# Sahar-E/NeRF-and-DietNeRF

Hardware: AMD Instinct MI355X
Metric: rays/sec (coarse+fine) at 256x256, 64 coarse + 128 fine samples (higher is better)
Workload: dtype f16 (3-pass hi/lo split operands, f32 accumulate; fp32-class results)

## Files before the change

nerf_and_dietnerf_amd/csrc/mlp_f16_frag.h:

```cpp
#pragma once
#include "mlp_common.h"

namespace nerf {

typedef _Float16 h8 __attribute__((ext_vector_type(8)));
typedef _Float16 h2 __attribute__((ext_vector_type(2)));
typedef uint32_t frag4 __attribute__((ext_vector_type(4)));

template <int OFF>
__device__ __forceinline__ void lds_read_frag_asm(f32x4& dst, uint32_t base) {
    asm volatile("ds_read_b128 %0, %1 offset:%2" : "=a"(dst) : "v"(base), "n"(OFF) : "memory");
}
template <int N>
__device__ __forceinline__ void lds_wait_frag_asm(f32x4& reg) {
#ifdef NERF_DIAG_NO_LDSWAIT
    asm volatile("" : "+a"(reg) : : "memory");
#else
    asm volatile("s_waitcnt lgkmcnt(%1)" : "+a"(reg) : "n"(N) : "memory");
#endif
}

__device__ __forceinline__ uint32_t pack_h2(float a, float b) {
    const h2 t = {(_Float16)a, (_Float16)b};
    return __builtin_bit_cast(uint32_t, t);
}

constexpr int kHCQ = 32;
constexpr int kHRing = 4;
constexpr int kHChunkBytes = kHCQ * kQuadBytes;
static_assert(kHRing * kHChunkBytes == kRingBytes, "fp16 ring must fill the shared LDS carve");

__device__ __forceinline__ void split_trunc(float y, float& hi_f, float& lo_f) {
    hi_f = __uint_as_float(__float_as_uint(y) & 0xFFFFE000u);
    lo_f = y - hi_f;
}


#ifndef NERF_PE_LX
#define NERF_PE_LX 5
#endif
constexpr int kPeLx = NERF_PE_LX;
constexpr int kPeDim = 3 + 6 * kPeLx;
constexpr int kHStepsPE = (kPeDim + 15) / 16;
constexpr int kHStepsHid = 16;
constexpr int kHStepsDir = 2;
constexpr int kHQpuPE = 2 * kHStepsPE;
constexpr int kHQpuHid = 2 * kHStepsHid;
constexpr int kHQpuSkip = kHQpuPE + kHQpuHid;
constexpr int kHQpuLast = kHQpuHid + 2 * kHStepsDir;
constexpr int kHTilesLast = 5;
constexpr int kHChunksPE = (8 * kHQpuPE + kHCQ - 1) / kHCQ;
constexpr int kHChunksHid = (8 * kHQpuHid) / kHCQ;
constexpr int kHChunksSkip = (8 * kHQpuSkip + kHCQ - 1) / kHCQ;
constexpr int kHChunksLast = (kHTilesLast * kHQpuLast + kHCQ - 1) / kHCQ;
constexpr int kHStreamChunks = kHChunksPE + 6 * kHChunksHid + kHChunksSkip + kHChunksLast;
constexpr int kHChunksSig = (kHQpuLast + kHCQ - 1) / kHCQ;
constexpr int kHStreamChunksSig = kHStreamChunks - kHChunksLast + kHChunksSig;
static_assert(kHStreamChunksSig * (size_t)kHChunkBytes == kStreamBytesF16Sig, "sigma-only stream size mismatch");
constexpr int kFChunksPE = (8 * kHStepsPE + kHCQ - 1) / kHCQ;
constexpr int kFChunksHid = (8 * kHStepsHid) / kHCQ;
constexpr int kFChunksSkip = (8 * (kHStepsPE + kHStepsHid) + kHCQ - 1) / kHCQ;
constexpr int kFChunksLast = (kHTilesLast * (kHStepsHid + kHStepsDir) + kHCQ - 1) / kHCQ;
constexpr int kFStreamChunks = kFChunksPE + 6 * kFChunksHid + kFChunksSkip + kFChunksLast;
static_assert(kFStreamChunks * (size_t)kHChunkBytes == kStreamBytesF16Hi, "hi-only stream size mismatch");
constexpr int kHConstBias = 0;
constexpr int kHConstBias8 = 2048;
constexpr int kHConstBiasSig = 2176;
constexpr int kHConstWrgb = 2208;
constexpr int kHConstBHead = 2592;
constexpr int kHConstFloats = 2608;

static_assert(kHStreamChunks * (size_t)kHChunkBytes == kStreamBytesF16, "stream size mismatch");
constexpr int kXChunksHidSig = (9 * kHQpuHid) / kHCQ;
constexpr int kXChunksLast0 = (4 * kHQpuHid) / kHCQ;
constexpr int kXStreamChunks = kHChunksPE + 6 * kHChunksHid + kHChunksSkip + kXChunksHidSig + kXChunksLast0;
constexpr int kXFChunksHidSig = (9 * kHStepsHid + kHCQ - 1) / kHCQ;
constexpr int kXFChunksLast0 = (4 * kHStepsHid) / kHCQ;
constexpr int kXFStreamChunks = kFChunksPE + 6 * kFChunksHid + kFChunksSkip + kXFChunksHidSig + kXFChunksLast0;
static_assert(kXStreamChunks * (size_t)kHChunkBytes == kStreamBytesF16Xyz, "xyz-only stream size mismatch");
static_assert(kXFStreamChunks * (size_t)kHChunkBytes == kStreamBytesF16HiXyz, "xyz-only hi stream size mismatch");
constexpr int kXConstBiasSig = 2048;
constexpr int kXConstBias8 = 2080;
constexpr int kXConstBias9 = 2336;
constexpr int kXConstWrgb = 2464;
constexpr int kXConstBHead = 2848;
constexpr int kXConstWsig = 2864;
constexpr int kXConstFloats = 3120;
static_assert(kXConstFloats <= kConstFloats, "xyz-only constants must fit the shared LDS carve");
enum { BODY_HIDSIG = 4, BODY_LAST0 = 5, BODY_SIG = 6 };
static_assert(kHConstFloats <= kConstFloats, "f16x3 constants must fit the shared LDS carve");

template <class T>
__device__ __forceinline__ void stream_store(T* p, const T& v) {
#ifndef NERF_STASH_NO_NT
    __builtin_nontemporal_store(v, p);
#else
    *p = v;
#endif
}
__device__ __forceinline__ void stream_store(uint2* p, const uint2& v) {
    typedef uint32_t u32x2 __attribute__((ext_vector_type(2)));
    u32x2 w;
    w[0] = v.x; w[1] = v.y;
    stream_store(reinterpret_cast<u32x2*>(p), w);
}

__device__ __forceinline__ uint32_t mask_push(uint32_t word, uint32_t packed_pair) {
    return (packed_pair & 0x80008000u) | (word >> 1);
}
__host__ __device__ constexpr int mask_bit(int ut, int r) { return 8 * (ut & 1) + (r >> 1) + 16 * (r & 1); }

__host__ __device__ inline int frag_feature(int n, int e, int h) {
    const int t = n >> 1, s = n & 1;
    return 32 * t + 16 * s + 8 * (e >> 2) + 4 * h + (e & 3);
}

}
```

nerf_and_dietnerf_amd/csrc/mlp_f16x3.hip:

```cpp
#include "mlp_f16_frag.h"

#include <math.h>
#include <string.h>

#if defined(NERF_BF16) && NERF_PE_LX == 5
namespace nerf::bf16 {
#elif defined(NERF_BF16)
namespace nerf::bf16::wide {
#elif NERF_PE_LX == 5
namespace nerf {
#else
namespace nerf::wide {
#endif

#ifdef NERF_BF16
typedef __bf16 e8 __attribute__((ext_vector_type(8)));
typedef __bf16 bf2 __attribute__((ext_vector_type(2)));
#define NERF_MFMA_E16 __builtin_amdgcn_mfma_f32_32x32x16_bf16
__device__ __forceinline__ void split_e(float y, float& hi_f, float& lo_f) {
    hi_f = __uint_as_float(__float_as_uint(y) & 0xFFFF0000u);
    lo_f = y - hi_f;
}
__device__ __forceinline__ uint32_t pack_hi(float a, float b) {
    return __builtin_amdgcn_perm(__float_as_uint(b), __float_as_uint(a), 0x07060302u);
}
__device__ __forceinline__ uint32_t pack_lo(float a, float b) {
    const bf2 t = {(__bf16)a, (__bf16)b};
    return __builtin_bit_cast(uint32_t, t);
}
#else
typedef h8 e8;
#define NERF_MFMA_E16 __builtin_amdgcn_mfma_f32_32x32x16_f16
__device__ __forceinline__ void split_e(float y, float& hi_f, float& lo_f) { split_trunc(y, hi_f, lo_f); }
__device__ __forceinline__ uint32_t pack_hi(float a, float b) { return pack_h2(a, b); }
__device__ __forceinline__ uint32_t pack_lo(float a, float b) { return pack_h2(a, b); }
#endif

#ifdef NERF_STAMPS
__device__ unsigned long long g_stamps_h[16];
#endif

template <int BODY, bool PENDING, bool FAST, bool STASH = false, int ROT = 0>
__device__ __forceinline__ void layer_body_h(Pipe& p, uint32_t lane16, uint32_t cb_h, int bias_off_bytes,
                                             float alpha, float* st_prev, float* st_cur, frag4* mk_prev_ptr,
                                             frag4* mk_cur_ptr, frag4& mk_prev, frag4& mk_cur, f32x16 (&accs)[4],
                                             frag4 (&xh)[16], frag4 (&xl)[16], frag4 (&nh)[14], frag4 (&nl)[14],
                                             const frag4 (&peh)[kHStepsPE], const frag4 (&pel)[kHStepsPE], const frag4 (&dh)[2],
                                             const frag4 (&dl)[2], float (&xc)[64], float& sigma_raw) {
    constexpr int NU = BODY == BODY_LAST ? kHTilesLast : BODY == BODY_SIG ? 1 : BODY == BODY_HIDSIG ? 9 : BODY == BODY_LAST0 ? 4 : 8;
    constexpr int NSTEP = BODY == BODY_PE ? kHStepsPE : (BODY == BODY_HID || BODY == BODY_HIDSIG || BODY == BODY_LAST0) ? kHStepsHid
                          : BODY == BODY_SKIP ? kHStepsPE + kHStepsHid : kHStepsHid + kHStepsDir;
    constexpr int SIG0 = BODY == BODY_HIDSIG ? 1 : 0;
    constexpr int TPS = FAST ? 1 : 2;
    constexpr int QPU = TPS * NSTEP;
    constexpr int NQ = NU * QPU;
#ifndef NERF_KPF
#define NERF_KPF 4
#endif
#ifndef NERF_KPF_FAST
#define NERF_KPF_FAST 8
#endif
    constexpr int kPf = FAST ? NERF_KPF_FAST : NERF_KPF;
#ifndef NERF_STASH_EXTRA_FAST
#define NERF_STASH_EXTRA_FAST 0
#endif
#ifndef NERF_STASH_EXTRA_3P
#define NERF_STASH_EXTRA_3P 0
#endif
    constexpr int kStashExtra = STASH ? (FAST ? NERF_STASH_EXTRA_FAST : NERF_STASH_EXTRA_3P) : 0;
    f32x4 pf[kPf];
    const int ck0 = p.ck;
    uint32_t rdbase[2];
    rdbase[0] = lane16 + (uint32_t)((ck0 + 0) & (kHRing - 1)) * kHChunkBytes;
    rdbase[1] = lane16 + (uint32_t)((ck0 + 1) & (kHRing - 1)) * kHChunkBytes;
    auto issue_read = [&](auto qc) {
        constexpr int Qa = decltype(qc)::value;
        lds_read_frag_asm<(Qa % kHCQ) * kQuadBytes>(pf[Qa % kPf], rdbase[(Qa / kHCQ) & 1]);
    };
    static_for<0, kPf>([&](auto ic) {
        if constexpr (decltype(ic)::value < NQ) issue_read(ic);
    });

    auto act = [&](float v) -> float {
        const float av = alpha * v;
        float y;
        asm("v_max_f32 %0, %1, %2" : "=v"(y) : "v"(v), "v"(av));
        return y;
    };
    auto load_bias = [&](int off_bytes, f32x16& dst) {
        static_for<0, 4>([&](auto gc) {
            constexpr int g = decltype(gc)::value;
            const f32x4 b = lds_read4(cb_h + off_bytes + g * 32);
            dst[4 * g + 0] = b[0]; dst[4 * g + 1] = b[1]; dst[4 * g + 2] = b[2]; dst[4 * g + 3] = b[3];
        });
    };
    float sq0 = 0.f, sq1 = 0.f;
    (void)sq0; (void)sq1;
    auto stash4 = [&](auto utc, auto rc, float y0, float y1, float* base) {
        constexpr int ut = decltype(utc)::value;
        constexpr int r = decltype(rc)::value;
        if constexpr ((r & 3) == 0) { sq0 = y0; sq1 = y1; }
        else {
            f32x4 v;
            v[0] = sq0; v[1] = sq1; v[2] = y0; v[3] = y1;
#ifndef NERF_DIAG_NO_STASH_STORES
            stream_store(reinterpret_cast<f32x4*>(base + 32 * (32 * ut + 8 * (r >> 2))), v);
#else
            asm volatile("" :: "v"(v), "v"(base));
#endif
        }
    };
    uint32_t sqh = 0u;
    (void)sqh;
    auto stash4h = [&](auto utc, auto rc, uint32_t ph, float* base) {
        constexpr int ut = decltype(utc)::value;
        constexpr int r = decltype(rc)::value;
        if constexpr ((r & 3) == 0) sqh = ph;
#ifndef NERF_DIAG_NO_STASH_STORES
        else stream_store(reinterpret_cast<uint2*>(reinterpret_cast<uint16_t*>(base) + 32 * (32 * ut + 8 * (r >> 2))), make_uint2(sqh, ph));
#else
        else asm volatile("" :: "v"(sqh), "v"(ph), "v"(base));
#endif
    };
    auto store_pair = [&](auto utc, auto rc, float y0, float y1, auto dest_sel, auto pend_sel) {
        constexpr int ut = decltype(utc)::value;
        constexpr int r = decltype(rc)::value;
        constexpr int n = 2 * ut + (r >> 3), e = r & 7;
        uint32_t ph, pl = 0u;
        if constexpr (FAST) {
            ph = pack_h2(y0, y1);
        } else {
            float h0, l0, h1, l1;
            split_e(y0, h0, l0);
            split_e(y1, h1, l1);
            ph = pack_hi(h0, h1); pl = pack_lo(l0, l1);
        }
        if constexpr (STASH) {
            if constexpr (FAST) stash4h(utc, rc, ph, decltype(pend_sel)::value ? st_prev : st_cur);
            else stash4(utc, rc, y0, y1, decltype(pend_sel)::value ? st_prev : st_cur);
            if constexpr (decltype(pend_sel)::value) mk_prev[ut >> 1] = mask_push(mk_prev[ut >> 1], ph);
            else mk_cur[ut >> 1] = mask_push(mk_cur[ut >> 1], ph);
        }
        if constexpr (decltype(dest_sel)::value) { xh[n][e >> 1] = ph; if constexpr (!FAST) xl[n][e >> 1] = pl; }
        else { nh[n][e >> 1] = ph; if constexpr (!FAST) nl[n][e >> 1] = pl; }
    };

#ifndef NERF_FAST_PACKED_EPI
#define NERF_FAST_PACKED_EPI 1
#endif
    constexpr bool kPackedEpi = FAST && NERF_FAST_PACKED_EPI != 0;
    const uint32_t alpha2 = pack_h2(alpha, alpha);
    (void)alpha2;
    auto act_pair = [&](float v0, float v1) -> uint32_t {
        const uint32_t pk = pack_h2(v0, v1);
        uint32_t q, y;
        asm("v_pk_mul_f16 %0, %1, %2" : "=v"(q) : "v"(pk), "v"(alpha2));
        asm("v_pk_max_f16 %0, %1, %2" : "=v"(y) : "v"(pk), "v"(q));
        return y;
    };
    auto store_pair_p = [&](auto utc, auto rc, uint32_t ph, auto dest_sel, auto pend_sel) {
        constexpr int ut = decltype(utc)::value;
        constexpr int r = decltype(rc)::value;
        constexpr int n = 2 * ut + (r >> 3), e = r & 7;
        if constexpr (STASH) {
            stash4h(utc, rc, ph, decltype(pend_sel)::value ? st_prev : st_cur);
            if constexpr (decltype(pend_sel)::value) mk_prev[ut >> 1] = mask_push(mk_prev[ut >> 1], ph);
            else mk_cur[ut >> 1] = mask_push(mk_cur[ut >> 1], ph);
        }
        if constexpr (decltype(dest_sel)::value) xh[n][e >> 1] = ph;
        else nh[n][e >> 1] = ph;
    };
    (void)act_pair; (void)store_pair_p;
    float ycarry = 0.f;
    (void)ycarry;
    static_for<0, NU>([&](auto uc) {
        constexpr int u = decltype(uc)::value;
        f32x16& acc = accs[(u + ROT) & 3];
        f32x16& prv = accs[(u + ROT + 3) & 3];
        f32x16& nxt = accs[(u + ROT + 1) & 3];
        if constexpr (u == 0 && !PENDING) load_bias(bias_off_bytes, acc);
        static_for<0, NSTEP>([&](auto nc) {
            constexpr int n = decltype(nc)::value;
            f32x4 araw[2];
            static_for<0, TPS>([&](auto tc) {
                constexpr int t = decltype(tc)::value;
                constexpr int Q = u * QPU + TPS * n + t;
                constexpr int left = NQ - Q;
                (void)left;
                constexpr int qc = Q % kHCQ;
                if constexpr (qc == 0 && Q > 0) p.ck += 1;
                if constexpr (qc == kHCQ / 2) {
                    constexpr int room = (NQ - 1 - Q) / 2;
                    pipe_sync_c<kHCQ, kHRing, (room + 1 < kHCQ / 4 ? room + 1 : kHCQ / 4), kStashExtra>(p);
                }
                if constexpr (qc > kHCQ / 2 && (qc - kHCQ / 2) % 2 == 0) {
                    constexpr int Qs = Q - (qc - kHCQ / 2);
                    constexpr bool tail = (NQ - 1 - Qs) / 2 + 1 < kHCQ / 4;
                    pipe_piece_c<(qc - kHCQ / 2) / 2, tail>(p);
                }
                lds_wait_frag_asm<(NQ - Q >= kPf ? kPf - 1 : NQ - Q - 1)>(pf[Q % kPf]);
                araw[t] = pf[Q % kPf];
                if constexpr (Q + kPf < NQ) {
                    constexpr int Qn = Q + kPf;
                    if constexpr (Qn % kHCQ == 0)
                        rdbase[(Qn / kHCQ) & 1] = lane16 + (uint32_t)((ck0 + Qn / kHCQ) & (kHRing - 1)) * kHChunkBytes;
                    issue_read(std::integral_constant<int, Qn>{});
                }
            });
            const e8 a_hi = __builtin_bit_cast(e8, araw[0]);
            const e8 a_lo = __builtin_bit_cast(e8, araw[FAST ? 0 : 1]);
            (void)a_lo;
            frag4 bh_, bl_;
            if constexpr (BODY == BODY_PE) { bh_ = peh[n]; bl_ = pel[n]; }
            else if constexpr (BODY == BODY_HID || BODY == BODY_HIDSIG || BODY == BODY_LAST0) { bh_ = xh[n]; bl_ = xl[n]; }
            else if constexpr (BODY == BODY_SKIP) {
                if constexpr (n < kHStepsPE) { bh_ = peh[n]; bl_ = pel[n]; }
                else { bh_ = xh[n - kHStepsPE]; bl_ = xl[n - kHStepsPE]; }
            } else {
                if constexpr (n < kHStepsHid) { bh_ = xh[n]; bl_ = xl[n]; }
                else { bh_ = dh[n - kHStepsHid]; bl_ = dl[n - kHStepsHid]; }
            }
            const e8 b_hi = __builtin_bit_cast(e8, bh_), b_lo = __builtin_bit_cast(e8, bl_);
            constexpr bool kPend = (u == 0) && PENDING && n < 8;
            constexpr bool kPrevS = (u > SIG0) && BODY != BODY_PE && NSTEP >= 16 && n < 16;
            constexpr int et = kPend ? 7 : (u > SIG0 ? u - 1 - SIG0 : 0);
            constexpr bool kXc = (BODY == BODY_LAST || BODY == BODY_LAST0) && kPrevS;
            if constexpr (BODY == BODY_HIDSIG && u == 1 && n == 0) sigma_raw = prv[0];
            if constexpr (!FAST) {
                acc = NERF_MFMA_E16(a_hi, b_lo, acc, 0, 0, 0);
                acc = NERF_MFMA_E16(a_lo, b_hi, acc, 0, 0, 0);
            }
            acc = NERF_MFMA_E16(a_hi, b_hi, acc, 0, 0, 0);
            if constexpr (kPend && kPackedEpi) {
                constexpr int er = 2 * n;
                store_pair_p(std::integral_constant<int, 7>{}, std::integral_constant<int, er>{}, act_pair(prv[er], prv[er + 1]), std::true_type{}, std::true_type{});
            } else if constexpr (kPrevS && !kXc && kPackedEpi) {
                if constexpr ((n & 1) == 1)
                    store_pair_p(std::integral_constant<int, et>{}, std::integral_constant<int, n - 1>{}, act_pair(prv[n - 1], prv[n]), std::false_type{}, std::false_type{});
            } else if constexpr (kPend) {
                constexpr int er = 2 * n;
                const float y0 = act(prv[er]), y1 = act(prv[er + 1]);
                store_pair(std::integral_constant<int, 7>{}, std::integral_constant<int, er>{}, y0, y1, std::true_type{}, std::true_type{});
            } else if constexpr (kPrevS) {
                const float y = act(prv[n]);
                if constexpr (kXc) {
                    xc[et * 16 + n] = y;
                    if constexpr (STASH) {
                        if constexpr ((n & 1) == 0) ycarry = y;
                        else {
                            const uint32_t pp = pack_h2(ycarry, y);
                            if constexpr (FAST) stash4h(std::integral_constant<int, et>{}, std::integral_constant<int, n - 1>{}, pp, st_cur);
                            else stash4(std::integral_constant<int, et>{}, std::integral_constant<int, n - 1>{}, ycarry, y, st_cur);
                            mk_cur[et >> 1] = mask_push(mk_cur[et >> 1], pp);
                        }
                    }
                }
                else if constexpr ((n & 1) == 0) ycarry = y;
                else store_pair(std::integral_constant<int, et>{}, std::integral_constant<int, n - 1>{}, ycarry, y, std::false_type{}, std::false_type{});
            }
            if constexpr (u == 0 && PENDING) {
                if constexpr (STASH && n == 8) { if (mk_prev_ptr) stream_store(mk_prev_ptr, mk_prev); }
                if constexpr (n == 8) { xh[12] = nh[12]; xl[12] = nl[12]; }
                if constexpr (n == 9) { xh[13] = nh[13]; xl[13] = nl[13]; }
            }
            if constexpr (n == (NSTEP >= 12 ? 10 : 0)) {
                if constexpr (u + 1 < NU) load_bias(bias_off_bytes + (u + 1) * 128, nxt);
                else if constexpr (BODY != BODY_LAST && BODY != BODY_LAST0 && BODY != BODY_SIG) load_bias(bias_off_bytes + NU * 128, nxt);
            }
            if constexpr (BODY == BODY_PE && u > 0 && n == 0) {
                static_for<0, 8>([&](auto pc) {
                    constexpr int r = 2 * decltype(pc)::value;
                    if constexpr (kPackedEpi) {
                        const uint32_t ph = act_pair(prv[r], prv[r + 1]);
                        if constexpr (u - 1 <= 5) store_pair_p(std::integral_constant<int, u - 1>{}, std::integral_constant<int, r>{}, ph, std::true_type{}, std::false_type{});
                        else store_pair_p(std::integral_constant<int, u - 1>{}, std::integral_constant<int, r>{}, ph, std::false_type{}, std::false_type{});
                        return;
                    }
                    const float z0 = act(prv[r]), z1 = act(prv[r + 1]);
                    if constexpr (u - 1 <= 5) store_pair(std::integral_constant<int, u - 1>{}, std::integral_constant<int, r>{}, z0, z1, std::true_type{}, std::false_type{});
                    else store_pair(std::integral_constant<int, u - 1>{}, std::integral_constant<int, r>{}, z0, z1, std::false_type{}, std::false_type{});
                });
            }
            if constexpr ((BODY == BODY_HID || BODY == BODY_SKIP || BODY == BODY_HIDSIG) && u == NU - 1) {
                constexpr int m = BODY == BODY_SKIP ? n - kHStepsPE : n;
                if constexpr (m >= 1 && m - 1 < 12) { xh[m - 1] = nh[m - 1]; xl[m - 1] = nl[m - 1]; }
            }
        });
    });
    if constexpr (BODY == BODY_LAST0) {
        f32x16& lastacc = accs[(NU - 1 + ROT) & 3];
#pragma unroll
        for (int r = 0; r < 16; ++r) xc[(NU - 1) * 16 + r] = act(lastacc[r]);
        if constexpr (STASH) {
            static_for<0, 8>([&](auto pc) {
                constexpr int r = 2 * decltype(pc)::value;
                const float y0 = xc[(NU - 1) * 16 + r], y1 = xc[(NU - 1) * 16 + r + 1];
                const uint32_t pp = pack_h2(y0, y1);
                if constexpr (FAST) stash4h(std::integral_constant<int, NU - 1>{}, std::integral_constant<int, r>{}, pp, st_cur);
                else stash4(std::integral_constant<int, NU - 1>{}, std::integral_constant<int, r>{}, y0, y1, st_cur);
                mk_cur[(NU - 1) >> 1] = mask_push(mk_cur[(NU - 1) >> 1], pp);
            });
            if (mk_cur_ptr) stream_store(mk_cur_ptr, mk_cur);
        }
    }
    if constexpr (BODY == BODY_LAST || BODY == BODY_SIG) {
        static_assert(((NU - 1 + ROT) & 3) == 0, "the sigma tile's accumulator");
        sigma_raw = accs[(NU - 1) & 3][0];
        if constexpr (STASH) { if (mk_cur_ptr) stream_store(mk_cur_ptr, mk_cur); }
    }
    if constexpr (NQ % kHCQ != 0 && NQ % kHCQ <= kHCQ / 2) pipe_sync_c<kHCQ, kHRing, 1, kStashExtra>(p);
    p.ck += 1;
}

template <bool FAST>
__device__ __forceinline__ void split8(const float (&v)[8], frag4& hi, frag4& lo) {
#pragma unroll
    for (int e = 0; e < 8; e += 2) {
        if constexpr (FAST) {
            hi[e >> 1] = pack_h2(v[e], v[e + 1]);
            lo[e >> 1] = 0u;
            continue;
        }
        float h0, l0, h1, l1;
        split_e(v[e], h0, l0);
        split_e(v[e + 1], h1, l1);
        hi[e >> 1] = pack_hi(h0, h1);
        lo[e >> 1] = pack_lo(l0, l1);
    }
}

template <bool FAST, bool STASH = false, bool XYZ = false, bool SIGONLY = false>
__device__ __forceinline__ void mlp_f16_body(const MlpArgs& a) {
    static_assert(!SIGONLY || (!FAST && !STASH && !XYZ), "the sigma-only variant is a render kernel of the 3-pass network");
    extern __shared__ __attribute__((aligned(16))) char smem[];
    const int tid = threadIdx.x;
    const int lane = tid & 63;
    const int wave = __builtin_amdgcn_readfirstlane(tid >> 6);
    const int j = lane & 31;
    const int h = lane >> 5;
    const uint32_t lane16 = kLdsRing + lane * 16;
    uint32_t cb_h = kLdsConst + h * 16;
    asm volatile("" : "+v"(cb_h));

    const long long ntiles = (a.M + 127) / 128;
    if ((long long)blockIdx.x >= ntiles) return;

    for (int i = tid; i < (XYZ ? kXConstFloats : kHConstFloats) / 4; i += 256) {
        const bool sig = SIGONLY && i >= kHConstBias8 / 4 && i < (kHConstBias8 + 32) / 4;
        reinterpret_cast<f32x4*>(smem + kLdsConst)[i] =
            reinterpret_cast<const f32x4*>(a.wconst)[sig ? i + (kHConstBiasSig - kHConstBias8) / 4 : i];
    }

    Pipe p;
    p.ck = 0;
    p.src_next = 0;
    p.n_chunks = XYZ ? (FAST ? kXFStreamChunks : kXStreamChunks) : SIGONLY ? kHStreamChunksSig : (FAST ? kFStreamChunks : kHStreamChunks);
    p.wbase = reinterpret_cast<const char*>(a.wstream);
    p.voff = wave * (kHCQ / 4 * kQuadBytes) + lane * 16;
    p.wave_lds = wave * (kHCQ / 4 * kQuadBytes);
    __syncthreads();
#pragma unroll
    for (int c = 0; c < kHRing - 1; ++c) {
        p.cur_src = p.wbase + (size_t)p.src_next * kHChunkBytes;
        p.cur_dst = kLdsRing + c * kHChunkBytes + p.wave_lds;
        p.src_next += 1;
#pragma unroll
        for (int j = 0; j < kHCQ / 4; ++j) dma_piece(p.cur_src, p.voff + j * kQuadBytes, p.cur_dst + j * kQuadBytes);
    }
    asm volatile("s_waitcnt vmcnt(%0)" ::"n"((kHCQ / 4) * (kHRing - 2)) : "memory");
    __builtin_amdgcn_s_barrier();
    asm volatile("" ::: "memory");

    frag4 xh[16], xl[16], nh[14], nl[14], peh[kHStepsPE], pel[kHStepsPE], dh[2], dl[2];
    f32x16 accs[4];
    float xc[64];
    float sigma_raw = 0.f;

    unsigned long long t0 = 0, t1 = 0, acc_t[8] = {0, 0, 0, 0, 0, 0, 0, 0};
    (void)t0; (void)t1; (void)acc_t;
    for (long long tile = blockIdx.x; tile < ntiles; tile += gridDim.x) {
        STAMP(t0);
        const long long m = tile * 128 + wave * 32 + j;
        const bool valid = m < a.M;
        const long long mm = valid ? m : a.M - 1;
        float px, py, pz, dx, dy, dz;
        if (a.mode == 0) {
            const long long ray = mm / a.S;
            const f32x4 o = *reinterpret_cast<const f32x4*>(a.in_a + ray * 4);
            const f32x4 d = *reinterpret_cast<const f32x4*>(a.in_b + ray * 4);
            const float zz = a.z[mm];
            px = __fadd_rn(o[0], __fmul_rn(d[0], zz));
            py = __fadd_rn(o[1], __fmul_rn(d[1], zz));
            pz = __fadd_rn(o[2], __fmul_rn(d[2], zz));
            dx = d[0]; dy = d[1]; dz = d[2];
        } else {
            px = a.in_a[mm * 3 + 0]; py = a.in_a[mm * 3 + 1]; pz = a.in_a[mm * 3 + 2];
            if constexpr (XYZ) { dx = dy = dz = 0.f; }
            else { dx = a.in_b[mm * 3 + 0]; dy = a.in_b[mm * 3 + 1]; dz = a.in_b[mm * 3 + 2]; }
        }
        const float kPi = 3.1415927410125732f;
        float pv[8 * kHStepsPE];
#pragma unroll
        for (int c = 0; c < 3; ++c) {
            const float v = c == 0 ? px : c == 1 ? py : pz;
            if constexpr (FAST) {
                sin_ladder_fp16_modes<kPeLx>(v * kPi, h, &pv[c * kPeLx]);
            } else {
#pragma unroll
                for (int k = 0; k < kPeLx; ++k) pv[c * kPeLx + k] = sin_shifted(v * (kPi * (float)(1 << k)), h);
            }
        }
        if constexpr (kPeLx == 5) {
            pv[15] = h ? 0.f : px; pv[16] = h ? 0.f : py; pv[17] = h ? 0.f : pz;
#pragma unroll
            for (int i = 18; i < 24; ++i) pv[i] = 0.f;
        } else {
            static_assert(kPeLx == 10, "the wide-PE layout holds exactly 10 octaves");
            pv[30] = h ? pz : px; pv[31] = h ? 0.f : py;
        }
#pragma unroll
        for (int n = 0; n < kHStepsPE; ++n) {
            float t8[8];
#pragma unroll
            for (int e = 0; e < 8; ++e) t8[e] = pv[n * 8 + e];
            split8<FAST>(t8, peh[n], pel[n]);
        }
        float dv[16];
#pragma unroll
        for (int c = 0; c < 3; ++c) {
            const float v = c == 0 ? dx : c == 1 ? dy : dz;
            if constexpr (FAST) {
                sin_ladder_fp16_modes<kLd>(v * kPi, h, &dv[c * kLd]);
            } else {
#pragma unroll
                for (int k = 0; k < kLd; ++k) dv[c * kLd + k] = sin_shifted(v * (kPi * (float)(1 << k)), h);
            }
        }
#pragma unroll
        for (int i = 12; i < 16; ++i) dv[i] = 0.f;
#pragma unroll
        for (int n = 0; n < 2; ++n) {
            float t8[8];
#pragma unroll
            for (int e = 0; e < 8; ++e) t8[e] = dv[n * 8 + e];
            split8<FAST>(t8, dh[n], dl[n]);
        }

        auto st_of = [&](int l) -> float* {
            if constexpr (!STASH) return nullptr;
            else {
                const long long row0 = a.diag_wrap ? (long long)(blockIdx.x & 63) * 128 + wave * 32 : tile * 128 + wave * 32;
                const long long off = row0 * (long long)a.st_ld[l] + (h * 32 + j) * 4;
                if constexpr (FAST) return reinterpret_cast<float*>(reinterpret_cast<uint16_t*>(a.st_ptr[l]) + off);
                else return a.st_ptr[l] + off;
            }
        };
        auto mk_of = [&](int l) -> frag4* {
            if constexpr (!STASH) return nullptr;
            else return a.mask_ptr[l] ? reinterpret_cast<frag4*>(a.mask_ptr[l]) + (tile * 128 + wave * 32 + j) * 2 + h
                                      : nullptr;
        };
        frag4 mk_prev = {0u, 0u, 0u, 0u}, mk_cur = {0u, 0u, 0u, 0u};
        frag4 *mk_prev_ptr = nullptr, *mk_cur_ptr = mk_of(0);
        float* st_prev = nullptr;
        float* st_cur = st_of(0);
        STAMP(t1); acc_t[0] += t1 - t0;
        layer_body_h<BODY_PE, false, FAST, STASH>(p, lane16, cb_h, (kHConstBias + 0 * 256) * 4, a.alpha, st_prev, st_cur, mk_prev_ptr, mk_cur_ptr, mk_prev, mk_cur, accs, xh, xl, nh, nl, peh, pel, dh, dl, xc, sigma_raw);
        STAMP(t0); acc_t[1] += t0 - t1;
#pragma unroll 1
        for (int l = 1; l <= 7; ++l) {
            st_prev = st_cur;
            st_cur = st_of(l);
            mk_prev_ptr = mk_cur_ptr; mk_cur_ptr = mk_of(l);
            mk_prev = mk_cur; mk_cur = frag4{0u, 0u, 0u, 0u};
            if (l == 4) {
                layer_body_h<BODY_SKIP, true, FAST, STASH>(p, lane16, cb_h, (kHConstBias + 4 * 256) * 4, a.alpha, st_prev, st_cur, mk_prev_ptr, mk_cur_ptr, mk_prev, mk_cur, accs, xh, xl, nh, nl, peh, pel, dh, dl, xc, sigma_raw);
                STAMP(t1); acc_t[3] += t1 - t0; t0 = t1;
            } else {
                layer_body_h<BODY_HID, true, FAST, STASH>(p, lane16, cb_h, (kHConstBias + l * 256) * 4, a.alpha, st_prev, st_cur, mk_prev_ptr, mk_cur_ptr, mk_prev, mk_cur, accs, xh, xl, nh, nl, peh, pel, dh, dl, xc, sigma_raw);
                STAMP(t1); acc_t[2] += t1 - t0; t0 = t1;
            }
        }
        if constexpr (XYZ) {
            st_prev = st_cur; st_cur = st_of(8);
            mk_prev_ptr = mk_cur_ptr; mk_cur_ptr = mk_of(8);
            mk_prev = mk_cur; mk_cur = frag4{0u, 0u, 0u, 0u};
            layer_body_h<BODY_HIDSIG, true, FAST, STASH, 0>(p, lane16, cb_h, kXConstBiasSig * 4, a.alpha, st_prev, st_cur, mk_prev_ptr, mk_cur_ptr, mk_prev, mk_cur, accs, xh, xl, nh, nl, peh, pel, dh, dl, xc, sigma_raw);
            st_prev = st_cur; st_cur = st_of(9);
            mk_prev_ptr = mk_cur_ptr; mk_cur_ptr = mk_of(9);
            mk_prev = mk_cur; mk_cur = frag4{0u, 0u, 0u, 0u};
            layer_body_h<BODY_LAST0, true, FAST, STASH, 1>(p, lane16, cb_h, kXConstBias9 * 4, a.alpha, st_prev, st_cur, mk_prev_ptr, mk_cur_ptr, mk_prev, mk_cur, accs, xh, xl, nh, nl, peh, pel, dh, dl, xc, sigma_raw);
        } else if constexpr (SIGONLY) {
            layer_body_h<BODY_SIG, true, FAST, STASH>(p, lane16, cb_h, kHConstBias8 * 4, a.alpha, st_prev, st_cur, mk_prev_ptr, mk_cur_ptr, mk_prev, mk_cur, accs, xh, xl, nh, nl, peh, pel, dh, dl, xc, sigma_raw);
            STAMP(t1); acc_t[4] += t1 - t0;
        } else {
            st_prev = st_cur;
            st_cur = st_of(8);
            mk_prev_ptr = mk_cur_ptr; mk_cur_ptr = mk_of(8);
            mk_prev = mk_cur; mk_cur = frag4{0u, 0u, 0u, 0u};
            layer_body_h<BODY_LAST, true, FAST, STASH>(p, lane16, cb_h, kHConstBias8 * 4, a.alpha, st_prev, st_cur, mk_prev_ptr, mk_cur_ptr, mk_prev, mk_cur, accs, xh, xl, nh, nl, peh, pel, dh, dl, xc, sigma_raw);
            STAMP(t1); acc_t[4] += t1 - t0;
        }
        if constexpr (SIGONLY) {
            if (valid && h == 0) {
                a.raw[m] = sigma_raw;
                if (a.nonfinite && !(fabsf(sigma_raw) <= 3.0e38f)) atomicAdd(a.nonfinite, 1ull);
            }
            STAMP(t0); acc_t[5] += t0 - t1; acc_t[6] += 1;
            continue;
        }
        float o0 = 0.f, o1 = 0.f, o2 = 0.f;
#pragma unroll
        for (int t = 0; t < 4; ++t) {
#pragma unroll
            for (int g = 0; g < 4; ++g) {
                constexpr int kW = XYZ ? kXConstWrgb : kHConstWrgb;
                const f32x4 w0 = lds_read4(cb_h + (kW + 0 * 128 + t * 32 + g * 8) * 4);
                const f32x4 w1 = lds_read4(cb_h + (kW + 1 * 128 + t * 32 + g * 8) * 4);
                const f32x4 w2 = lds_read4(cb_h + (kW + 2 * 128 + t * 32 + g * 8) * 4);
#pragma unroll
                for (int e = 0; e < 4; ++e) {
                    const float x = xc[t * 16 + g * 4 + e];
                    o0 = fmaf(w0[e], x, o0);
                    o1 = fmaf(w1[e], x, o1);
                    o2 = fmaf(w2[e], x, o2);
                }
            }
        }
        o0 += __shfl_xor(o0, 32);
        o1 += __shfl_xor(o1, 32);
        o2 += __shfl_xor(o2, 32);
        const f32x4 bh = lds_read4(kLdsConst + (XYZ ? kXConstBHead : kHConstBHead) * 4);
        if (valid && h == 0) {
            f32x4 out;
            out[0] = o0 + bh[0]; out[1] = o1 + bh[1]; out[2] = o2 + bh[2]; out[3] = sigma_raw;
            *reinterpret_cast<f32x4*>(a.raw + m * 4) = out;
            const float chk = out[0] + out[1] + out[2] + out[3];
            if (a.nonfinite && !(fabsf(chk) <= 3.0e38f)) atomicAdd(a.nonfinite, 1ull);
        }
        STAMP(t0); acc_t[5] += t0 - t1; acc_t[6] += 1;
    }
#ifdef NERF_STAMPS
    if (blockIdx.x == 0 && tid == 0)
        for (int i = 0; i < 8; ++i) g_stamps_h[i] = acc_t[i];
#endif
    asm volatile("s_waitcnt vmcnt(0)" ::: "memory");
}

#ifdef NERF_BF16
__global__ __launch_bounds__(256, 1) void mlp_bf16x3_kernel(const MlpArgs a) { mlp_f16_body<false>(a); }
__global__ __launch_bounds__(256, 1) void mlp_bf16x3_xyz_kernel(const MlpArgs a) { mlp_f16_body<false, false, true>(a); }
#if NERF_PE_LX == 5
__global__ __launch_bounds__(256, 1) void mlp_bf16x3_sig_kernel(const MlpArgs a) { mlp_f16_body<false, false, false, true>(a); }
#endif

static int bf_grid(const MlpArgs& a, int num_cus) {
    const long long ntiles = (a.M + 127) / 128;
    return (int)(ntiles < (long long)num_cus ? ntiles : (long long)num_cus);
}
void launch_mlp_bf16x3(const MlpArgs& a, int num_cus, hipStream_t stream, bool xyz_only) {
    if (a.M <= 0) return;
    if (xyz_only) hipLaunchKernelGGL(mlp_bf16x3_xyz_kernel, dim3(bf_grid(a, num_cus)), dim3(256), kLdsTotal, stream, a);
    else hipLaunchKernelGGL(mlp_bf16x3_kernel, dim3(bf_grid(a, num_cus)), dim3(256), kLdsTotal, stream, a);
}
#if NERF_PE_LX == 5
void launch_mlp_bf16x3_sig(const MlpArgs& a, int num_cus, hipStream_t stream) {
    if (a.M <= 0) return;
    hipLaunchKernelGGL(mlp_bf16x3_sig_kernel, dim3(bf_grid(a, num_cus)), dim3(256), kLdsTotal, stream, a);
}
#endif
void mlp_bf16x3_set_attributes() {
    (void)hipFuncSetAttribute(reinterpret_cast<const void*>(mlp_bf16x3_kernel),
                              hipFuncAttributeMaxDynamicSharedMemorySize, kLdsTotal);
    (void)hipFuncSetAttribute(reinterpret_cast<const void*>(mlp_bf16x3_xyz_kernel),
                              hipFuncAttributeMaxDynamicSharedMemorySize, kLdsTotal);
#if NERF_PE_LX == 5
    (void)hipFuncSetAttribute(reinterpret_cast<const void*>(mlp_bf16x3_sig_kernel),
                              hipFuncAttributeMaxDynamicSharedMemorySize, kLdsTotal);
#endif
}
#else
__global__ __launch_bounds__(256, 1) void mlp_f16x3_kernel(const MlpArgs a) { mlp_f16_body<false>(a); }
__global__ __launch_bounds__(256, 1) void mlp_f16_kernel(const MlpArgs a) { mlp_f16_body<true>(a); }
__global__ __launch_bounds__(256, 1) void mlp_f16x3_stash_kernel(const MlpArgs a) { mlp_f16_body<false, true>(a); }
__global__ __launch_bounds__(256, 1) void mlp_f16_stash_kernel(const MlpArgs a) { mlp_f16_body<true, true>(a); }
__global__ __launch_bounds__(256, 1) void mlp_f16x3_xyz_kernel(const MlpArgs a) { mlp_f16_body<false, false, true>(a); }
#if NERF_PE_LX == 5
__global__ __launch_bounds__(256, 1) void mlp_f16x3_sig_kernel(const MlpArgs a) { mlp_f16_body<false, false, false, true>(a); }
#endif
__global__ __launch_bounds__(256, 1) void mlp_f16_xyz_kernel(const MlpArgs a) { mlp_f16_body<true, false, true>(a); }
__global__ __launch_bounds__(256, 1) void mlp_f16x3_xyz_stash_kernel(const MlpArgs a) { mlp_f16_body<false, true, true>(a); }
__global__ __launch_bounds__(256, 1) void mlp_f16_xyz_stash_kernel(const MlpArgs a) { mlp_f16_body<true, true, true>(a); }

void launch_mlp_f16x3_stash(const MlpArgs& a, int num_cus, hipStream_t stream, bool single_pass, bool xyz_only) {
    if (a.M <= 0) return;
    const long long ntiles = (a.M + 127) / 128;
    const int grid = (int)(ntiles < (long long)num_cus ? ntiles : (long long)num_cus);
    if (xyz_only) {
        if (single_pass) hipLaunchKernelGGL(mlp_f16_xyz_stash_kernel, dim3(grid), dim3(256), kLdsTotal, stream, a);
        else hipLaunchKernelGGL(mlp_f16x3_xyz_stash_kernel, dim3(grid), dim3(256), kLdsTotal, stream, a);
        return;
    }
    if (single_pass) hipLaunchKernelGGL(mlp_f16_stash_kernel, dim3(grid), dim3(256), kLdsTotal, stream, a);
    else hipLaunchKernelGGL(mlp_f16x3_stash_kernel, dim3(grid), dim3(256), kLdsTotal, stream, a);
}

void launch_mlp_f16x3(const MlpArgs& a, int num_cus, hipStream_t stream, bool single_pass, bool xyz_only) {
    if (a.M <= 0) return;
    const long long ntiles = (a.M + 127) / 128;
    const int grid = (int)(ntiles < (long long)num_cus ? ntiles : (long long)num_cus);
    if (xyz_only) {
        if (single_pass) hipLaunchKernelGGL(mlp_f16_xyz_kernel, dim3(grid), dim3(256), kLdsTotal, stream, a);
        else hipLaunchKernelGGL(mlp_f16x3_xyz_kernel, dim3(grid), dim3(256), kLdsTotal, stream, a);
        return;
    }
    if (single_pass) hipLaunchKernelGGL(mlp_f16_kernel, dim3(grid), dim3(256), kLdsTotal, stream, a);
    else hipLaunchKernelGGL(mlp_f16x3_kernel, dim3(grid), dim3(256), kLdsTotal, stream, a);
}

#if NERF_PE_LX == 5
void launch_mlp_f16x3_sig(const MlpArgs& a, int num_cus, hipStream_t stream) {
    if (a.M <= 0) return;
    const long long ntiles = (a.M + 127) / 128;
    const int grid = (int)(ntiles < (long long)num_cus ? ntiles : (long long)num_cus);
    hipLaunchKernelGGL(mlp_f16x3_sig_kernel, dim3(grid), dim3(256), kLdsTotal, stream, a);
}
#endif

#if defined(NERF_STAMPS) && NERF_PE_LX == 5
extern "C" void nerf_debug_read_stamps_h(unsigned long long* out) {
    (void)hipDeviceSynchronize();
    (void)hipMemcpyFromSymbol(out, HIP_SYMBOL(g_stamps_h), sizeof(unsigned long long) * 16);
}
#endif

void mlp_f16x3_set_attributes() {
    (void)hipFuncSetAttribute(reinterpret_cast<const void*>(mlp_f16x3_kernel),
                              hipFuncAttributeMaxDynamicSharedMemorySize, kLdsTotal);
    (void)hipFuncSetAttribute(reinterpret_cast<const void*>(mlp_f16_kernel),
                              hipFuncAttributeMaxDynamicSharedMemorySize, kLdsTotal);
    (void)hipFuncSetAttribute(reinterpret_cast<const void*>(mlp_f16x3_stash_kernel),
                              hipFuncAttributeMaxDynamicSharedMemorySize, kLdsTotal);
    (void)hipFuncSetAttribute(reinterpret_cast<const void*>(mlp_f16_stash_kernel),
                              hipFuncAttributeMaxDynamicSharedMemorySize, kLdsTotal);
    (void)hipFuncSetAttribute(reinterpret_cast<const void*>(mlp_f16x3_xyz_kernel),
                              hipFuncAttributeMaxDynamicSharedMemorySize, kLdsTotal);
    (void)hipFuncSetAttribute(reinterpret_cast<const void*>(mlp_f16_xyz_kernel),
                              hipFuncAttributeMaxDynamicSharedMemorySize, kLdsTotal);
    (void)hipFuncSetAttribute(reinterpret_cast<const void*>(mlp_f16x3_xyz_stash_kernel),
                              hipFuncAttributeMaxDynamicSharedMemorySize, kLdsTotal);
    (void)hipFuncSetAttribute(reinterpret_cast<const void*>(mlp_f16_xyz_stash_kernel),
                              hipFuncAttributeMaxDynamicSharedMemorySize, kLdsTotal);
#if NERF_PE_LX == 5
    (void)hipFuncSetAttribute(reinterpret_cast<const void*>(mlp_f16x3_sig_kernel),
                              hipFuncAttributeMaxDynamicSharedMemorySize, kLdsTotal);
#endif
}
#endif

namespace {
uint16_t f32_to_f16(float f) {
    uint32_t x;
    memcpy(&x, &f, 4);
    const uint32_t sign = (x >> 16) & 0x8000u;
    x &= 0x7FFFFFFFu;
    if (x >= 0x7F800000u) return (uint16_t)(sign | 0x7C00u | (x > 0x7F800000u ? 0x200u : 0));
    if (x >= 0x477FF000u) return (uint16_t)(sign | 0x7C00u);
    if (x < 0x33000001u) return (uint16_t)sign;
    int e = (int)(x >> 23) - 127;
    uint32_t m = (x & 0x7FFFFFu) | 0x800000u;
    int shift;
    uint32_t base;
    if (e < -14) { shift = 13 + (-14 - e); base = 0; }
    else { shift = 13; base = (uint32_t)(e + 15) << 10; m &= 0x7FFFFFu; }
    uint32_t q = m >> shift;
    const uint32_t rem = m & ((1u << shift) - 1), halfway = 1u << (shift - 1);
    if (rem > halfway || (rem == halfway && (q & 1))) q += 1;
    return (uint16_t)(sign | (base + q));
}
float f16_to_f32(uint16_t hbits) {
    const uint32_t sign = (uint32_t)(hbits & 0x8000u) << 16;
    const uint32_t e = (hbits >> 10) & 0x1F, m = hbits & 0x3FF;
    uint32_t x;
    if (e == 0) {
        if (m == 0) x = sign;
        else { float f = (float)m * 5.9604644775390625e-08f; memcpy(&x, &f, 4); x |= sign; }
    } else if (e == 31) x = sign | 0x7F800000u | (m << 13);
    else x = sign | ((e + 112) << 23) | (m << 13);
    float f;
    memcpy(&f, &x, 4);
    return f;
}
#ifdef NERF_BF16
uint16_t f32_to_e16(float f) {
    uint32_t x;
    memcpy(&x, &f, 4);
    if ((x & 0x7FFFFFFFu) > 0x7F800000u) return (uint16_t)((x >> 16) | 0x40u);
    return (uint16_t)((x + 0x7FFFu + ((x >> 16) & 1u)) >> 16);
}
float e16_to_f32(uint16_t b) {
    const uint32_t x = (uint32_t)b << 16;
    float f;
    memcpy(&f, &x, 4);
    return f;
}
#else
uint16_t f32_to_e16(float f) { return f32_to_f16(f); }
float e16_to_f32(uint16_t hbits) { return f16_to_f32(hbits); }
#endif
int h_pe_row(int v, int h) {
    if (v < 3 * kPeLx) { const int c = v / kPeLx, k = v % kPeLx; return c * (1 + 2 * kPeLx) + 1 + 2 * k + h; }
    if (kPeLx != 5) {
        if (v == 30) return h ? 2 * (1 + 2 * kPeLx) : 0;
        return v == 31 && h == 0 ? 1 + 2 * kPeLx : -1;
    }
    if (v < 18 && h == 0) return (v - 15) * 11;
    return -1;
}
int h_hid_row(int n, int e, int h) { const int t = n >> 1, s = n & 1; return 32 * t + 16 * s + 8 * (e >> 2) + 4 * h + (e & 3); }
int h_dir_row(int v, int h, int n_angles) {
    if (v >= 12) return -1;
    const int c = v / 4, k = v % 4;
    if (n_angles == 2) return c * 8 + 2 * k + h;
    if (c == 1) return -1;
    return (c == 0 ? 0 : 1) * 8 + 2 * k + h;
}
struct HLayer { const float* k; const float* b; int in, out; };
}

template <class EmitW, class EmitC>
static void pack_f16_map(int n_angles, bool hi_only, EmitW emit_w, EmitC emit_c, bool sig_only = false) {
    const int kd = 256 + 8 * (n_angles + 1);
    const bool xyz_only = n_angles == 0;
    const int shapes_dir[12][2] = {{kPeDim, 256}, {256, 256}, {256, 256}, {256, 256}, {kPeDim + 256, 256}, {256, 256},
                                   {256, 256}, {256, 256}, {kd, 128}, {128, 3}, {kd, 1}, {0, 0}};
    const int shapes_xyz[12][2] = {{kPeDim, 256}, {256, 256}, {256, 256}, {256, 256}, {kPeDim + 256, 256}, {256, 256},
                                   {256, 256}, {256, 256}, {256, 256}, {256, 128}, {128, 3}, {256, 1}};
    const int (*shapes)[2] = xyz_only ? shapes_xyz : shapes_dir;
    struct Lay { long long k, b; int in, out; } L[12];
    long long off = 0;
    for (int i = 0; i < (xyz_only ? 12 : 11); ++i) {
        L[i].in = shapes[i][0]; L[i].out = shapes[i][1];
        L[i].k = off; off += (long long)L[i].in * L[i].out;
        L[i].b = off; off += L[i].out;
    }
    size_t chunk = 0;
    auto emit_body = [&](int layer, int body) {
        const int NU = body == BODY_LAST ? kHTilesLast : body == BODY_SIG ? 1 : body == BODY_HIDSIG ? 9 : body == BODY_LAST0 ? 4 : 8;
        const int NSTEP = body == BODY_PE ? kHStepsPE : (body == BODY_HID || body == BODY_HIDSIG || body == BODY_LAST0) ? kHStepsHid
                          : body == BODY_SKIP ? kHStepsPE + kHStepsHid : kHStepsHid + kHStepsDir;
        const long long b0 = (long long)chunk * (kHChunkBytes / 2);
        for (int u = 0; u < NU; ++u)
            for (int n = 0; n < NSTEP; ++n)
                for (int lane = 0; lane < 64; ++lane)
                    for (int e = 0; e < 8; ++e) {
                        const int i = lane & 31, h = lane >> 5;
                        int row;
                        if (body == BODY_PE) row = h_pe_row(n * 8 + e, h);
                        else if (body == BODY_HID || body == BODY_HIDSIG || body == BODY_LAST0) row = h_hid_row(n, e, h);
                        else if (body == BODY_SKIP) {
                            if (n < kHStepsPE) row = h_pe_row(n * 8 + e, h);
                            else row = kPeDim + h_hid_row(n - kHStepsPE, e, h);
                        } else {
                            if (n < kHStepsHid) row = h_hid_row(n, e, h);
                            else { const int r = h_dir_row((n - kHStepsHid) * 8 + e, h, n_angles); row = r < 0 ? -1 : kHidden + r; }
                        }
                        long long src = -1;
                        if (row >= 0) {
                            if ((body == BODY_LAST && u == kHTilesLast - 1) || body == BODY_SIG)
                                src = i == 0 ? L[10].k + row : -1;
                            else if (body == BODY_HIDSIG && u == 0) src = i == 0 ? L[11].k + row : -1;
                            else if (body == BODY_HIDSIG) src = L[layer].k + (long long)row * L[layer].out + 32 * (u - 1) + i;
                            else src = L[layer].k + (long long)row * L[layer].out + 32 * u + i;
                        }
                        if (hi_only) {
                            emit_w(b0 + (long long)(u * NSTEP + n) * (kQuadBytes / 2) + lane * 8 + e, -1LL, src);
                        } else {
                            const long long q = (long long)(u * NSTEP + n) * 2;
                            emit_w(b0 + (q + 0) * (kQuadBytes / 2) + lane * 8 + e, b0 + (q + 1) * (kQuadBytes / 2) + lane * 8 + e, src);
                        }
                    }
        chunk += (NU * NSTEP * (hi_only ? 1 : 2) + kHCQ - 1) / kHCQ;
    };
    emit_body(0, BODY_PE);
    for (int l = 1; l <= 3; ++l) emit_body(l, BODY_HID);
    emit_body(4, BODY_SKIP);
    for (int l = 5; l <= 7; ++l) emit_body(l, BODY_HID);
    for (int l = 0; l < 8; ++l)
        for (int f = 0; f < 256; ++f) emit_c(kHConstBias + l * 256 + f, L[l].b + f);
    if (xyz_only) {
        emit_body(8, BODY_HIDSIG);
        emit_body(9, BODY_LAST0);
        emit_c(kXConstBiasSig + 0, L[11].b);
        for (int f = 0; f < 256; ++f) emit_c(kXConstBias8 + f, L[8].b + f);
        for (int f = 0; f < 128; ++f) emit_c(kXConstBias9 + f, L[9].b + f);
        for (int c = 0; c < 3; ++c)
            for (int f = 0; f < 128; ++f) emit_c(kXConstWrgb + c * 128 + f, L[10].k + f * 3 + c);
        for (int c = 0; c < 3; ++c) emit_c(kXConstBHead + c, L[10].b + c);
        for (int f = 0; f < 256; ++f) emit_c(kXConstWsig + f, L[11].k + f);
        return;
    }
    emit_body(8, sig_only ? BODY_SIG : BODY_LAST);
    for (int f = 0; f < 128; ++f) emit_c(kHConstBias8 + f, L[8].b + f);
    emit_c(kHConstBiasSig + 0, L[10].b);
    for (int c = 0; c < 3; ++c)
        for (int f = 0; f < 128; ++f) emit_c(kHConstWrgb + c * 128 + f, L[9].k + f * 3 + c);
    for (int c = 0; c < 3; ++c) emit_c(kHConstBHead + c, L[9].b + c);
}

static void pack_weights_f16_impl(const float* blob, int n_angles, void* stream_out, float* const_out, bool hi_only,
                                  bool sig_only = false) {
    memset(stream_out, 0, sig_only ? kStreamBytesF16Sig : n_angles == 0 ? (hi_only ? kStreamBytesF16HiXyz : kStreamBytesF16Xyz)
                                                                        : (hi_only ? kStreamBytesF16Hi : kStreamBytesF16));
    memset(const_out, 0, kConstBytes);
    uint16_t* base = reinterpret_cast<uint16_t*>(stream_out);
    pack_f16_map(n_angles, hi_only,
                 [&](long long ph, long long pl, long long src) {
                     const float w = src < 0 ? 0.f : blob[src];
                     const uint16_t hi = f32_to_e16(w);
                     base[ph] = hi;
                     if (pl >= 0) base[pl] = f32_to_e16(w - e16_to_f32(hi));
                 },
                 [&](long long pos, long long src) { const_out[pos] = blob[src]; }, sig_only);
}

#if defined(NERF_BF16) && NERF_PE_LX == 5
__global__ void repack_bf16x3_kernel(const float* __restrict__ blob, const int32_t* __restrict__ stream_idx,
                                     uint16_t* __restrict__ stream, size_t n_slots) {
    const size_t i = (size_t)blockIdx.x * blockDim.x + threadIdx.x;
    if (i >= n_slots) return;
    const int32_t t = stream_idx[i];
    uint16_t out = 0;
    if (t != 0) {
        const float w = blob[(t >> 1) - 1];
        const __bf16 hi = (__bf16)w;
        const __bf16 v = (t & 1) ? (__bf16)(w - (float)hi) : hi;
        out = __builtin_bit_cast(uint16_t, v);
    }
    stream[i] = out;
}
void launch_repack_bf16x3(const float* blob, const int32_t* stream_idx, void* stream, size_t stream_bytes, hipStream_t s) {
    const size_t n = stream_bytes / 2;
    hipLaunchKernelGGL(repack_bf16x3_kernel, dim3((unsigned)((n + 255) / 256)), dim3(256), 0, s, blob, stream_idx,
                       reinterpret_cast<uint16_t*>(stream), n);
}
void pack_weights_bf16x3_sig(const float* blob, int n_angles, void* stream_out, float* const_out) {
    pack_weights_f16_impl(blob, n_angles, stream_out, const_out, false, true);
}
#endif
#ifdef NERF_BF16
void pack_weights_bf16x3(const float* blob, int n_angles, void* stream_out, float* const_out) {
    pack_weights_f16_impl(blob, n_angles, stream_out, const_out, false);
}
#else
size_t f16_stream_bytes(int n_angles, bool hi_only) {
    if (n_angles == 0) return hi_only ? kStreamBytesF16HiXyz : kStreamBytesF16Xyz;
    return hi_only ? kStreamBytesF16Hi : kStreamBytesF16;
}

void build_f16x3_gather(int n_angles, bool hi_only, int32_t* stream_idx ,
                        int32_t* const_idx ) {
    memset(stream_idx, 0, (f16_stream_bytes(n_angles, hi_only) / 2) * sizeof(int32_t));
    memset(const_idx, 0, kConstFloats * sizeof(int32_t));
    pack_f16_map(n_angles, hi_only,
                 [&](long long ph, long long pl, long long src) {
                     if (src < 0) return;
                     stream_idx[ph] = (int32_t)(2 * (src + 1));
                     if (pl >= 0) stream_idx[pl] = (int32_t)(2 * (src + 1) + 1);
                 },
                 [&](long long pos, long long src) { const_idx[pos] = (int32_t)(src + 1); });
}

__global__ void repack_f16x3_kernel(const float* __restrict__ blob, const int32_t* __restrict__ stream_idx,
                                    uint16_t* __restrict__ stream, const int32_t* __restrict__ const_idx,
                                    float* __restrict__ cst, size_t n_slots) {
    const size_t i = (size_t)blockIdx.x * blockDim.x + threadIdx.x;
    if (i < n_slots) {
        const int32_t t = stream_idx[i];
        uint16_t out = 0;
        if (t != 0) {
            const float w = blob[(t >> 1) - 1];
            const _Float16 hi = (_Float16)w;
            const _Float16 v = (t & 1) ? (_Float16)(w - (float)hi) : hi;
            out = __builtin_bit_cast(uint16_t, v);
        }
        stream[i] = out;
    }
    if (i < (size_t)kConstFloats) {
        const int32_t t = const_idx[i];
        cst[i] = t ? blob[t - 1] : 0.f;
    }
}

void launch_repack_f16x3(const float* blob, const int32_t* stream_idx, void* stream, const int32_t* const_idx, float* cst,
                         size_t stream_bytes, hipStream_t s) {
    const size_t n = stream_bytes / 2;
    hipLaunchKernelGGL(repack_f16x3_kernel, dim3((unsigned)((n + 255) / 256)), dim3(256), 0, s, blob, stream_idx,
                       reinterpret_cast<uint16_t*>(stream), const_idx, cst, n);
}

void pack_weights_f16x3(const float* blob, int n_angles, void* stream_out, float* const_out) {
    pack_weights_f16_impl(blob, n_angles, stream_out, const_out, false);
}
void pack_weights_f16(const float* blob, int n_angles, void* stream_out, float* const_out) {
    pack_weights_f16_impl(blob, n_angles, stream_out, const_out, true);
}
#if NERF_PE_LX == 5
void pack_weights_f16x3_sig(const float* blob, int n_angles, void* stream_out, float* const_out) {
    pack_weights_f16_impl(blob, n_angles, stream_out, const_out, false, true);
}
void build_f16x3_sig_gather(int n_angles, int32_t* stream_idx) {
    memset(stream_idx, 0, (kStreamBytesF16Sig / 2) * sizeof(int32_t));
    pack_f16_map(n_angles, false,
                 [&](long long ph, long long pl, long long src) {
                     if (src < 0) return;
                     stream_idx[ph] = (int32_t)(2 * (src + 1));
                     stream_idx[pl] = (int32_t)(2 * (src + 1) + 1);
                 },
                 [](long long, long long) {}, true);
}
#endif
#endif

}
```

nerf_and_dietnerf_amd/csrc/nerf_api.hip:

```cpp
#include "../../include/nerf_mi355.h"

#include <stdarg.h>
#include <stdio.h>
#include <stdlib.h>
#include <string.h>

#include <algorithm>
#include <string>
#include <vector>

#include "nerf_ctx.h"

using namespace nerf;

thread_local std::string g_err;

namespace nerf {

int fail(const char* fmt, ...) {
    char buf[512];
    va_list ap;
    va_start(ap, fmt);
    vsnprintf(buf, sizeof buf, fmt, ap);
    va_end(ap);
    g_err = buf;
    return 1;
}

int ensure(nerf_ctx* c, DevBuf& b, size_t bytes) {
    if (bytes <= b.cap) return 0;
    HIP_OK(hipStreamSynchronize(c->stream));
    if (b.p) HIP_OK(hipFree(b.p));
    b.p = nullptr; b.cap = 0;
    size_t want = bytes + bytes / 8;
    HIP_OK(hipMalloc(&b.p, want));
    b.cap = want;
    return 0;
}

int h2d(nerf_ctx* c, DevBuf& b, const void* src, size_t bytes) {
    if (int r = ensure(c, b, bytes)) return r;
    HIP_OK(hipMemcpyAsync(b.p, src, bytes, hipMemcpyHostToDevice, c->stream));
    return 0;
}

int enter(nerf_ctx* c) {
    if (!c) return fail("ctx is NULL");
    HIP_OK(hipSetDevice(c->cfg.device));
    return 0;
}

int sampling_ok(const nerf_ctx* c) {
    if (c->sampling == NERF_SAMPLING_LINDISP && !(c->cfg.near_boundary > 0.f)) return fail("lindisp needs near_boundary > 0");
    return 0;
}

static int layer_dims(int lx, int ld, int n_angles, int dims[12][2]) {
    const int xd = 3 + 6 * lx;
    const int kd = 256 + 2 * ld * (n_angles + 1);
    const int with_dirs[11][2] = {{xd, 256}, {256, 256}, {256, 256}, {256, 256}, {xd + 256, 256}, {256, 256},
                                  {256, 256}, {256, 256}, {kd, 128}, {128, 3}, {kd, 1}};
    const int xyz_only[12][2] = {{xd, 256}, {256, 256}, {256, 256}, {256, 256}, {xd + 256, 256}, {256, 256},
                                 {256, 256}, {256, 256}, {256, 256}, {256, 128}, {128, 3}, {256, 1}};
    const int n = n_angles == 0 ? 12 : 11;
    for (int l = 0; l < n; ++l) {
        dims[l][0] = n_angles == 0 ? xyz_only[l][0] : with_dirs[l][0];
        dims[l][1] = n_angles == 0 ? xyz_only[l][1] : with_dirs[l][1];
    }
    return n;
}

size_t blob_floats(int lx, int ld, int n_angles) {
    int dims[12][2];
    const int n = layer_dims(lx, ld, n_angles, dims);
    size_t s = 0;
    for (int l = 0; l < n; ++l) s += (size_t)dims[l][0] * dims[l][1] + dims[l][1];
    return s;
}

void blob_expand_index(int lx, int ld, int n_angles, int32_t* idx, int layout_lx) {
    int wide[12][2], dims[12][2];
    const int n = layer_dims(layout_lx, kLd, n_angles, wide);
    layer_dims(lx, ld, n_angles, dims);
    const int xd_layout = 3 + 6 * layout_lx;
    auto xyz_row = [&](int r) {
        const int c = r / (1 + 2 * layout_lx), j = r % (1 + 2 * layout_lx);
        if (j == 0) return c * (1 + 2 * lx);
        const int k = (j - 1) / 2, h = (j - 1) % 2;
        return k < lx ? c * (1 + 2 * lx) + 1 + 2 * k + h : -1;
    };
    auto dir_row = [&](int r) {
        const int c = r / (2 * kLd), j = r % (2 * kLd), k = j / 2, h = j % 2;
        return k < ld ? c * 2 * ld + 2 * k + h : -1;
    };
    size_t src = 0, dst = 0;
    for (int l = 0; l < n; ++l) {
        for (int r = 0; r < wide[l][0]; ++r) {
            int rs = r;
            if (l == 0) rs = xyz_row(r);
            else if (l == 4) rs = r < xd_layout ? xyz_row(r) : 3 + 6 * lx + (r - xd_layout);
            else if (n_angles != 0 && (l == 8 || l == 10)) rs = r < kHidden ? r : (dir_row(r - kHidden) < 0 ? -1 : kHidden + dir_row(r - kHidden));
            for (int f = 0; f < wide[l][1]; ++f)
                idx[dst++] = rs < 0 ? 0 : (int32_t)(src + (size_t)rs * dims[l][1] + f + 1);
        }
        src += (size_t)dims[l][0] * dims[l][1];
        for (int f = 0; f < wide[l][1]; ++f) idx[dst++] = (int32_t)(src + f + 1);
        src += dims[l][1];
    }
}

int upload_packed_weights(nerf_ctx* c, int which, const float* blob_in) {
    HIP_OK(hipSetDevice(c->cfg.device));
    NetWeights& n = c->net[which];
    std::vector<float> spread;
    const float* blob = blob_in;
    const int L = pe_layout_lx(c->cfg.n_pos_enc_xyz);
    if (c->cfg.n_pos_enc_xyz != L || c->cfg.n_pos_enc_dir != kLd) {
        std::vector<int32_t> idx(blob_floats(L, kLd, c->cfg.n_angles));
        blob_expand_index(c->cfg.n_pos_enc_xyz, c->cfg.n_pos_enc_dir, c->cfg.n_angles, idx.data(), L);
        spread.resize(idx.size());
        for (size_t i = 0; i < idx.size(); ++i) spread[i] = idx[i] ? blob_in[idx[i] - 1] : 0.f;
        blob = spread.data();
    }
    StreamDesc d[kStreamKinds];
    render_streams(c->cfg.n_pos_enc_xyz, c->cfg.n_angles, which, d);
    std::vector<float> cst[kConstBlocks];
    bool drained = false;
    for (int k = 0; k < kStreamKinds; ++k) {
        if (!d[k].bytes) continue;
        std::vector<char> host(d[k].bytes);
        cst[d[k].cst].resize(kConstFloats);
        d[k].pack(blob, c->cfg.n_angles, host.data(), cst[d[k].cst].data());
        if (!n.stream[k]) HIP_OK(hipMalloc(&n.stream[k], d[k].bytes));
        if (!drained) HIP_OK(hipStreamSynchronize(c->stream));
        drained = true;
        HIP_OK(hipMemcpy(n.stream[k], host.data(), d[k].bytes, hipMemcpyHostToDevice));
    }
    for (int b = 0; b < kConstBlocks; ++b) {
        if (cst[b].empty()) continue;
        if (!n.cst[b]) HIP_OK(hipMalloc((void**)&n.cst[b], kConstBytes));
        HIP_OK(hipMemcpy(n.cst[b], cst[b].data(), kConstBytes, hipMemcpyHostToDevice));
    }
    const size_t nf = nerf_blob_size(&c->cfg);
    if (n.host_blob.data() != blob_in) n.host_blob.assign(blob_in, blob_in + nf);
    n.loaded = true;
    return 0;
}

}

namespace {

struct RenderKernel {
    StreamKind stream;
    ConstBlock cst;
    void (*launch)(const MlpArgs& a, int num_cus, hipStream_t s, bool xyz_only);
    bool sigma_only;
};
int pick_render_kernel(const nerf_config& cfg, int precision, bool want_sigma, RenderKernel* k) {
    const bool wide_pe = cfg.n_pos_enc_xyz > kLx, sig = want_sigma && !wide_pe && cfg.n_angles != 0;
    switch (precision) {
    case NERF_PRECISION_FP32:
        if (wide_pe)
            return fail("n_pos_enc_dim_xyz %d (> %d) renders with the 16-bit-core kernels only: precision f16x3, bf16x3 or f16, not fp32",
                        cfg.n_pos_enc_xyz, kLx);
        *k = {kFp32, kConstFp32, [](const MlpArgs& a, int n, hipStream_t s, bool x) { launch_mlp_fp32(a, n, s, x); }, false};
        return 0;
    case NERF_PRECISION_F16X3:
        if (sig) *k = {kF16x3Sig, kConst16, [](const MlpArgs& a, int n, hipStream_t s, bool) { launch_mlp_f16x3_sig(a, n, s); }, true};
        else if (wide_pe) *k = {kF16x3, kConst16, [](const MlpArgs& a, int n, hipStream_t s, bool x) { wide::launch_mlp_f16x3(a, n, s, false, x); }, false};
        else *k = {kF16x3, kConst16, [](const MlpArgs& a, int n, hipStream_t s, bool x) { launch_mlp_f16x3(a, n, s, false, x); }, false};
        return 0;
    case NERF_PRECISION_F16: {
        static const bool one_tile = [] { const char* e = getenv("NERF_F16_TILES"); return e && e[0] == '1'; }();
        if (wide_pe) *k = {kF16Hi, kConst16, [](const MlpArgs& a, int n, hipStream_t s, bool x) { wide::launch_mlp_f16x3(a, n, s, true, x); }, false};
        else if (cfg.n_angles != 0 && !one_tile) *k = {kF16Hi, kConst16, [](const MlpArgs& a, int n, hipStream_t s, bool) { launch_mlp_f16_2t(a, n, s); }, false};
        else *k = {kF16Hi, kConst16, [](const MlpArgs& a, int n, hipStream_t s, bool x) { launch_mlp_f16x3(a, n, s, true, x); }, false};
        return 0;
    }
    case NERF_PRECISION_BF16X3:
        if (sig) *k = {kBf16x3Sig, kConst16, [](const MlpArgs& a, int n, hipStream_t s, bool) { bf16::launch_mlp_bf16x3_sig(a, n, s); }, true};
        else if (wide_pe) *k = {kBf16x3, kConst16, [](const MlpArgs& a, int n, hipStream_t s, bool x) { bf16::wide::launch_mlp_bf16x3(a, n, s, x); }, false};
        else *k = {kBf16x3, kConst16, [](const MlpArgs& a, int n, hipStream_t s, bool x) { bf16::launch_mlp_bf16x3(a, n, s, x); }, false};
        return 0;
    }
    fail("unknown precision %d", precision);
    return 2;
}

int check_cfg(const nerf_config* cfg) {
    if (!cfg) return fail("nerf_config is NULL");
    if (cfg->n_angles != 2 && cfg->n_angles != 1 && cfg->n_angles != 0)
        return fail("n_angles_for_model should be 1 or 2.");
    if (cfg->n_pos_enc_xyz < 1 || cfg->n_pos_enc_xyz > kLxWide || cfg->n_pos_enc_dir < 1 || cfg->n_pos_enc_dir > kLd ||
        cfg->hidden_dim != kHidden || cfg->last_hidden_dim != kLast)
        return fail("supported networks: n_pos_enc_dim_xyz 1..%d, n_pos_enc_view_dir 1..%d, hidden %d, last hidden %d "
                    "(got %d %d %d %d)", kLxWide, kLd, kHidden, kLast, cfg->n_pos_enc_xyz, cfg->n_pos_enc_dir, cfg->hidden_dim,
                    cfg->last_hidden_dim);
    RenderKernel k;
    if (pick_render_kernel(*cfg, cfg->precision, false, &k) == 2)
        return fail("unknown precision %d (NERF_PRECISION_FP32 = 0, NERF_PRECISION_F16X3 = 1, NERF_PRECISION_F16 = 2, "
                    "NERF_PRECISION_BF16X3 = 3)", cfg->precision);
    return 0;
}

int run_mlp(nerf_ctx* c, int which, const RenderKernel& k, const float* in_a, const float* in_b, const float* z, float* raw,
            long long M, int S, int mode) {
    if (!c->net[which].loaded) return fail("network %d has no weights loaded", which);
    if (int r = train_flush_weights(c, which)) return r;
    MlpArgs a{};
    a.wstream = (const float*)c->net[which].stream[k.stream];
    a.wconst = c->net[which].cst[k.cst];
    if (!a.wstream || !a.wconst) return fail("internal: network %d keeps no stream of kind %d", which, (int)k.stream);
    a.in_a = in_a; a.in_b = in_b; a.z = z; a.raw = raw; a.M = M; a.S = S; a.mode = mode;
    a.nonfinite = c->nonfinite;
    a.alpha = c->cfg.leaky_relu_alpha;
    hipEvent_t e0 = nullptr, e1 = nullptr;
    if (c->timing) {
        if (c->ev_used == c->ev_pool.size()) {
            hipEvent_t x, y;
            HIP_OK(hipEventCreate(&x));
            HIP_OK(hipEventCreate(&y));
            c->ev_pool.emplace_back(x, y);
        }
        e0 = c->ev_pool[c->ev_used].first; e1 = c->ev_pool[c->ev_used].second;
        c->ev_used++;
        c->timed_rows += M;
        HIP_OK(hipEventRecord(e0, c->stream));
    }
    k.launch(a, c->num_cus, c->stream, c->cfg.n_angles == 0);
    if (c->timing) HIP_OK(hipEventRecord(e1, c->stream));
    HIP_OK(hipGetLastError());
    return 0;
}

struct OutSizes { size_t per_ray[7]; };
OutSizes out_sizes(int S) {
    OutSizes o;
    o.per_ray[0] = 3; o.per_ray[1] = S; o.per_ray[2] = S; o.per_ray[3] = S; o.per_ray[4] = 3 * (size_t)S;
    o.per_ray[5] = S; o.per_ray[6] = 1;
    return o;
}
float** out_ptrs(nerf_outputs& o, int i) {
    switch (i) {
        case 0: return &o.rgb; case 1: return &o.weights; case 2: return &o.cumprod; case 3: return &o.alpha;
        case 4: return &o.rgb_samples; case 5: return &o.z; default: return &o.depth;
    }
}

int make_dev_outputs(nerf_ctx* c, const nerf_outputs* host, long long N, int S, nerf_outputs* dev) {
    const OutSizes sz = out_sizes(S);
    nerf_outputs h = host ? *host : nerf_outputs{};
    *dev = nerf_outputs{};
    for (int i = 0; i < 7; ++i) {
        if (!*out_ptrs(h, i)) continue;
        if (int r = ensure(c, c->b_out[i], sz.per_ray[i] * N * sizeof(float))) return r;
        *out_ptrs(*dev, i) = (float*)c->b_out[i].p;
    }
    return 0;
}
int copy_back_outputs(nerf_ctx* c, const nerf_outputs* host, const nerf_outputs* dev, long long N, int S) {
    const OutSizes sz = out_sizes(S);
    nerf_outputs h = host ? *host : nerf_outputs{};
    nerf_outputs d = *dev;
    for (int i = 0; i < 7; ++i) {
        float* hp = *out_ptrs(h, i);
        if (!hp) continue;
        HIP_OK(hipMemcpyAsync(hp, *out_ptrs(d, i), sz.per_ray[i] * N * sizeof(float), hipMemcpyDeviceToHost,
                              c->stream));
    }
    HIP_OK(hipStreamSynchronize(c->stream));
    return 0;
}

int copy_back_batch(nerf_ctx* c, const nerf_outputs* host, const nerf_outputs* dev, long long off, long long n, int S,
                    size_t batch_index) {
    if (!c->copy_stream) HIP_OK(hipStreamCreateWithFlags(&c->copy_stream, hipStreamNonBlocking));
    constexpr size_t kRing = 64;
    if (c->copy_ev.size() < kRing) {
        hipEvent_t e;
        HIP_OK(hipEventCreateWithFlags(&e, hipEventDisableTiming));
        c->copy_ev.push_back(e);
    }
    hipEvent_t ev = c->copy_ev[batch_index % c->copy_ev.size()];
    HIP_OK(hipEventRecord(ev, c->stream));
    HIP_OK(hipStreamWaitEvent(c->copy_stream, ev, 0));
    const OutSizes sz = out_sizes(S);
    nerf_outputs h = host ? *host : nerf_outputs{};
    nerf_outputs d = *dev;
    for (int i = 0; i < 7; ++i) {
        float* hp = *out_ptrs(h, i);
        if (!hp) continue;
        HIP_OK(hipMemcpyAsync(hp + sz.per_ray[i] * off, *out_ptrs(d, i) + sz.per_ray[i] * off,
                              sz.per_ray[i] * n * sizeof(float), hipMemcpyDeviceToHost, c->copy_stream));
    }
    return 0;
}

int dev_render_rays(nerf_ctx* c, int which, const float* o, const float* d, const float* z, long long N, int S,
                    const nerf_outputs& outs) {
    const bool weights_only = outs.weights && !outs.rgb && !outs.cumprod && !outs.alpha && !outs.rgb_samples && !outs.z &&
                              !outs.depth;
    RenderKernel k;
    if (pick_render_kernel(c->cfg, c->cfg.precision, which == NERF_NET_COARSE && weights_only, &k)) return 1;
    if (k.sigma_only) {
        if (int r = ensure(c, c->b_raw, (size_t)N * S * sizeof(float))) return r;
        float* sigma = (float*)c->b_raw.p;
        if (int r = run_mlp(c, which, k, o, d, z, sigma, N * S, S, 0)) return r;
        launch_composite_weights(sigma, z, N, S, outs.weights, c->stream);
        HIP_OK(hipGetLastError());
        return 0;
    }
    if (int r = ensure(c, c->b_raw, (size_t)N * S * 4 * sizeof(float))) return r;
    float* raw = (float*)c->b_raw.p;
    if (int r = run_mlp(c, which, k, o, d, z, raw, N * S, S, 0)) return r;
    launch_composite(raw, z, N, S, outs.rgb, outs.weights, outs.cumprod, outs.alpha, outs.rgb_samples, outs.depth,
                     c->stream);
    if (outs.z && outs.z != z)
        HIP_OK(hipMemcpyAsync(outs.z, z, (size_t)N * S * sizeof(float), hipMemcpyDeviceToDevice, c->stream));
    HIP_OK(hipGetLastError());
    return 0;
}

int dev_render(nerf_ctx* c, const float* o, const float* d, long long N, int Sc, int Sf, const float* u_c,
               const float* u_f, uint64_t seed, long long ray_base, const nerf_outputs& outs) {
    const bool fine = Sf > 0 && c->net[NERF_NET_FINE].loaded;
    if (int r = sampling_ok(c)) return r;
    if (int r = ensure(c, c->b_zc, (size_t)N * Sc * sizeof(float))) return r;
    float* zc = (float*)c->b_zc.p;
    launch_z_values(c->cfg.near_boundary, c->cfg.far_boundary, c->sampling == NERF_SAMPLING_LINDISP, N, Sc, u_c, seed, ray_base,
                    zc, c->stream);
    if (!fine) return dev_render_rays(c, NERF_NET_COARSE, o, d, zc, N, Sc, outs);
    if (Sc < 2) return fail("hierarchical sampling needs at least 2 coarse samples (got %d)", Sc);
    if (int r = ensure(c, c->b_wc, (size_t)N * Sc * sizeof(float))) return r;
    nerf_outputs co{};
    co.weights = (float*)c->b_wc.p;
    if (int r = dev_render_rays(c, NERF_NET_COARSE, o, d, zc, N, Sc, co)) return r;
    const int St = Sc + Sf;
    if (int r = ensure(c, c->b_zf, (size_t)N * St * sizeof(float))) return r;
    float* zf = (float*)c->b_zf.p;
    launch_sample_pdf(co.weights, zc, N, Sc, Sf, u_f, seed, ray_base, nullptr, zf, c->stream);
    return dev_render_rays(c, NERF_NET_FINE, o, d, zf, N, St, outs);
}

}

extern "C" {

int nerf_abi_version(void) { return NERF_ABI_VERSION; }
const char* nerf_last_error(void) { return g_err.c_str(); }

size_t nerf_blob_size(const nerf_config* cfg) {
    if (check_cfg(cfg)) return 0;
    return blob_floats(cfg->n_pos_enc_xyz, cfg->n_pos_enc_dir, cfg->n_angles);
}

int nerf_ctx_create(const nerf_config* cfg, nerf_ctx** out) {
    if (!out) return fail("out is NULL");
    *out = nullptr;
    if (int r = check_cfg(cfg)) return r;
    RenderKernel k;
    if (pick_render_kernel(*cfg, cfg->precision, false, &k)) return 1;
    int ndev = 0;
    hipError_t e = hipGetDeviceCount(&ndev);
    if (e != hipSuccess || ndev == 0)
        return fail("no HIP device available (%s): libnerf_mi355 has no CPU path", hipGetErrorString(e));
    if (cfg->device < 0 || cfg->device >= ndev) return fail("device %d out of range (%d devices)", cfg->device, ndev);
    HIP_OK(hipSetDevice(cfg->device));
    hipDeviceProp_t prop;
    HIP_OK(hipGetDeviceProperties(&prop, cfg->device));
    if (strncmp(prop.gcnArchName, "gfx950", 6) != 0)
        return fail("device %d is %s; this library is built for gfx950 (MI355X) only", cfg->device, prop.gcnArchName);
    nerf_ctx* c = new nerf_ctx();
    c->cfg = *cfg;
    c->num_cus = prop.multiProcessorCount;
    if (hipStreamCreateWithFlags(&c->own_stream, hipStreamNonBlocking) != hipSuccess) {
        delete c;
        return fail("hipStreamCreate failed");
    }
    c->stream = c->own_stream;
    if (hipMalloc((void**)&c->nonfinite, sizeof(unsigned long long)) != hipSuccess ||
        hipMemset(c->nonfinite, 0, sizeof(unsigned long long)) != hipSuccess) {
        delete c;
        return fail("hipMalloc of the status counter failed");
    }
    mlp_fp32_set_attributes();
    mlp_f16x3_set_attributes();
    wide::mlp_f16x3_set_attributes();
    bf16::mlp_bf16x3_set_attributes();
    bf16::wide::mlp_bf16x3_set_attributes();
    mlp_bwd_f16x3_set_attributes();
    mlp_f16_2t_set_attributes();
    *out = c;
    return 0;
}

void nerf_ctx_destroy(nerf_ctx* c) {
    if (!c) return;
    (void)hipSetDevice(c->cfg.device);
    (void)hipStreamSynchronize(c->stream);
    DevBuf* bufs[] = {&c->b_orig, &c->b_dirs, &c->b_zc, &c->b_zf, &c->b_raw, &c->b_wc, &c->b_u0, &c->b_u1,
                      &c->b_in0, &c->b_in1, &c->b_in2};
    for (DevBuf* b : bufs) if (b->p) (void)hipFree(b->p);
    for (auto& b : c->b_out) if (b.p) (void)hipFree(b.p);
    for (auto& n : c->net) {
        for (void* p : n.stream) if (p) (void)hipFree(p);
        for (float* p : n.cst) if (p) (void)hipFree(p);
    }
    for (auto& ev : c->ev_pool) { (void)hipEventDestroy(ev.first); (void)hipEventDestroy(ev.second); }
    if (c->copy_stream) { (void)hipStreamSynchronize(c->copy_stream); (void)hipStreamDestroy(c->copy_stream); }
    for (hipEvent_t e : c->copy_ev) (void)hipEventDestroy(e);
    comm_free(c);
    train_free(c);
    if (c->nonfinite) (void)hipFree(c->nonfinite);
    if (c->own_stream) (void)hipStreamDestroy(c->own_stream);
    delete c;
}

int nerf_ctx_synchronize(nerf_ctx* c) {
    if (!c) return fail("ctx is NULL");
    HIP_OK(hipStreamSynchronize(c->stream));
    return 0;
}

int nerf_ctx_set_stream(nerf_ctx* c, void* s) {
    if (!c) return fail("ctx is NULL");
    HIP_OK(hipStreamSynchronize(c->stream));
    c->stream = (s == NERF_STREAM_OWN) ? c->own_stream : (hipStream_t)s;
    return 0;
}

int nerf_ctx_set_bounds(nerf_ctx* c, float near_b, float far_b) {
    if (!c) return fail("ctx is NULL");
    c->cfg.near_boundary = near_b; c->cfg.far_boundary = far_b;
    return 0;
}

int nerf_ctx_set_sampling(nerf_ctx* c, int mode) {
    if (!c) return fail("ctx is NULL");
    if (mode != NERF_SAMPLING_LINEAR && mode != NERF_SAMPLING_LINDISP)
        return fail("unknown sampling mode %d (NERF_SAMPLING_LINEAR = 0, NERF_SAMPLING_LINDISP = 1)", mode);
    if (mode == NERF_SAMPLING_LINDISP && !(c->cfg.near_boundary > 0.f)) return fail("lindisp needs near_boundary > 0");
    c->sampling = mode;
    return 0;
}

int nerf_ctx_set_ray_space(nerf_ctx* c, int space, float ndc_near_plane) {
    if (!c) return fail("ctx is NULL");
    if (space != NERF_RAYS_WORLD && space != NERF_RAYS_NDC)
        return fail("unknown ray space %d (NERF_RAYS_WORLD = 0, NERF_RAYS_NDC = 1)", space);
    if (space == NERF_RAYS_NDC && !(ndc_near_plane > 0.f)) return fail("ndc_near_plane must be > 0 (got %g)", ndc_near_plane);
    c->ray_space = space;
    if (space == NERF_RAYS_NDC) c->ndc_near_plane = ndc_near_plane;
    return 0;
}

int nerf_ctx_set_precision(nerf_ctx* c, int precision) {
    if (!c) return fail("ctx is NULL");
    RenderKernel k;
    if (pick_render_kernel(c->cfg, precision, false, &k)) return 1;
    HIP_OK(hipStreamSynchronize(c->stream));
    c->cfg.precision = precision;
    return 0;
}

int nerf_load_weights(nerf_ctx* c, int which, const float* blob, size_t n_floats) {
    if (!c || !blob) return fail("ctx/blob is NULL");
    if (which != NERF_NET_COARSE && which != NERF_NET_FINE) return fail("which must be 0 (coarse) or 1 (fine)");
    const size_t want = nerf_blob_size(&c->cfg);
    if (n_floats != want) return fail("weight blob has %zu floats, expected %zu", n_floats, want);
    if (int r = upload_packed_weights(c, which, blob)) return r;
    return train_on_load(c, which);
}

int nerf_get_rays_directions(nerf_ctx* c, const float* c2w, float fov, int32_t H, int32_t W, float* dirs, int mem) {
    ENTER(c);
    if (!c || !c2w || !dirs) return fail("NULL argument");
    if (H <= 0 || W <= 0) return fail("bad image size %dx%d", H, W);
    const long long N = (long long)H * W;
    float* d = dirs;
    if (mem == NERF_MEM_HOST) {
        if (int r = ensure(c, c->b_dirs, N * 16)) return r;
        d = (float*)c->b_dirs.p;
    }
    launch_raygen(c2w, fov, H, W, 0, N, nullptr, d, c->stream);
    HIP_OK(hipGetLastError());
    if (mem == NERF_MEM_HOST) {
        HIP_OK(hipMemcpyAsync(dirs, d, N * 16, hipMemcpyDeviceToHost, c->stream));
        HIP_OK(hipStreamSynchronize(c->stream));
    }
    return 0;
}

int nerf_rays_to_ndc(nerf_ctx* c, const float* rays_orig, const float* rays_dirs, int64_t N, float fov, float ndc_near_plane,
                     float* out_orig, float* out_dirs, int mem) {
    ENTER(c);
    if (!rays_orig || !rays_dirs || !out_orig || !out_dirs) return fail("NULL argument");
    if (N < 0) return fail("bad shape N=%lld", (long long)N);
    if (!(ndc_near_plane > 0.f)) return fail("ndc_near_plane must be > 0 (got %g)", ndc_near_plane);
    if ((out_orig == rays_orig) != (out_dirs == rays_dirs) || out_orig == rays_dirs || out_dirs == rays_orig || out_orig == out_dirs)
        return fail("nerf_rays_to_ndc works in place only as out_orig == rays_orig AND out_dirs == rays_dirs");
    if (N == 0) return 0;
    const float *o = rays_orig, *d = rays_dirs;
    float *oo = out_orig, *od = out_dirs;
    if (mem == NERF_MEM_HOST) {
        if (int r = h2d(c, c->b_orig, rays_orig, (size_t)N * 16)) return r;
        if (int r = h2d(c, c->b_dirs, rays_dirs, (size_t)N * 16)) return r;
        o = oo = (float*)c->b_orig.p; d = od = (float*)c->b_dirs.p;
    }
    launch_rays_to_ndc(o, d, N, fov, ndc_near_plane, oo, od, c->stream);
    HIP_OK(hipGetLastError());
    if (mem == NERF_MEM_HOST) {
        HIP_OK(hipMemcpyAsync(out_orig, oo, (size_t)N * 16, hipMemcpyDeviceToHost, c->stream));
        HIP_OK(hipMemcpyAsync(out_dirs, od, (size_t)N * 16, hipMemcpyDeviceToHost, c->stream));
        HIP_OK(hipStreamSynchronize(c->stream));
    }
    return 0;
}

int nerf_get_z_values(nerf_ctx* c, int64_t N, int32_t S, const float* u, uint64_t seed, int64_t ray_base, float* z,
                      int mem) {
    ENTER(c);
    if (!c || !z) return fail("NULL argument");
    if (N < 0 || S <= 0) return fail("bad shape N=%lld S=%d", (long long)N, S);
    if (int r = sampling_ok(c)) return r;
    const float* du = u;
    float* dz = z;
    if (mem == NERF_MEM_HOST) {
        if (u) { if (int r = h2d(c, c->b_u0, u, (size_t)N * S * 4)) return r; du = (const float*)c->b_u0.p; }
        if (int r = ensure(c, c->b_zc, (size_t)N * S * 4)) return r;
        dz = (float*)c->b_zc.p;
    }
    launch_z_values(c->cfg.near_boundary, c->cfg.far_boundary, c->sampling == NERF_SAMPLING_LINDISP, N, S, du, seed, ray_base,
                    dz, c->stream);
    HIP_OK(hipGetLastError());
    if (mem == NERF_MEM_HOST) {
        HIP_OK(hipMemcpyAsync(z, dz, (size_t)N * S * 4, hipMemcpyDeviceToHost, c->stream));
        HIP_OK(hipStreamSynchronize(c->stream));
    }
    return 0;
}

int nerf_sample_pdf(nerf_ctx* c, const float* weights, const float* z, int64_t N, int32_t S, int32_t Sf,
                    const float* u, uint64_t seed, int64_t ray_base, float* z_new, float* z_merged, int mem) {
    ENTER(c);
    if (!c || !weights || !z) return fail("NULL argument");
    if (N < 0 || S < 2 || Sf <= 0) return fail("bad shape N=%lld S=%d Sf=%d (need S>=2, Sf>=1)", (long long)N, S, Sf);
    if (sample_pdf_lds_bytes(S, Sf) > 64 * 1024) return fail("S=%d Sf=%d exceeds the sampler's LDS budget", S, Sf);
    const float *dw = weights, *dz = z, *du = u;
    float *dn = z_new, *dm = z_merged;
    if (mem == NERF_MEM_HOST) {
        if (int r = h2d(c, c->b_in0, weights, (size_t)N * S * 4)) return r;
        if (int r = h2d(c, c->b_in1, z, (size_t)N * S * 4)) return r;
        dw = (const float*)c->b_in0.p; dz = (const float*)c->b_in1.p;
        if (u) { if (int r = h2d(c, c->b_u1, u, (size_t)N * Sf * 4)) return r; du = (const float*)c->b_u1.p; }
        if (z_new) { if (int r = ensure(c, c->b_in2, (size_t)N * Sf * 4)) return r; dn = (float*)c->b_in2.p; }
        if (z_merged) { if (int r = ensure(c, c->b_zf, (size_t)N * (S + Sf) * 4)) return r; dm = (float*)c->b_zf.p; }
    }
    launch_sample_pdf(dw, dz, N, S, Sf, du, seed, ray_base, dn, dm, c->stream);
    HIP_OK(hipGetLastError());
    if (mem == NERF_MEM_HOST) {
        if (z_new) HIP_OK(hipMemcpyAsync(z_new, dn, (size_t)N * Sf * 4, hipMemcpyDeviceToHost, c->stream));
        if (z_merged) HIP_OK(hipMemcpyAsync(z_merged, dm, (size_t)N * (S + Sf) * 4, hipMemcpyDeviceToHost, c->stream));
        HIP_OK(hipStreamSynchronize(c->stream));
    }
    return 0;
}

int nerf_positional_encoding(nerf_ctx* c, const float* x, int64_t M, int32_t n_enc, int32_t passthrough, float* out,
                             int mem) {
    ENTER(c);
    if (!c || !x || !out) return fail("NULL argument");
    if (M < 0 || n_enc < 0 || n_enc > 16) return fail("bad shape M=%lld n_enc=%d", (long long)M, n_enc);
    const size_t per = 3 * ((passthrough ? 1 : 0) + 2 * (size_t)n_enc);
    const float* dx = x;
    float* dout = out;
    if (mem == NERF_MEM_HOST) {
        if (int r = h2d(c, c->b_in0, x, (size_t)M * 12)) return r;
        if (int r = ensure(c, c->b_in1, (size_t)M * per * 4)) return r;
        dx = (const float*)c->b_in0.p; dout = (float*)c->b_in1.p;
    }
    launch_posenc(dx, M, n_enc, passthrough, dout, c->stream);
    HIP_OK(hipGetLastError());
    if (mem == NERF_MEM_HOST) {
        HIP_OK(hipMemcpyAsync(out, dout, (size_t)M * per * 4, hipMemcpyDeviceToHost, c->stream));
        HIP_OK(hipStreamSynchronize(c->stream));
    }
    return 0;
}

int nerf_model_predict(nerf_ctx* c, int which, const float* xyz, const float* view_dirs, int64_t M, float* raw,
                       int mem) {
    ENTER(c);
    if (!c || !xyz || !raw || (!view_dirs && c->cfg.n_angles != 0)) return fail("NULL argument");
    if (which != 0 && which != 1) return fail("which must be 0 (coarse) or 1 (fine)");
    if (M < 0) return fail("bad M");
    const float *dx = xyz, *dv = view_dirs;
    float* dr = raw;
    if (mem == NERF_MEM_HOST) {
        if (int r = h2d(c, c->b_in0, xyz, (size_t)M * 12)) return r;
        if (view_dirs)
            if (int r = h2d(c, c->b_in1, view_dirs, (size_t)M * 12)) return r;
        if (int r = ensure(c, c->b_raw, (size_t)M * 16)) return r;
        dx = (const float*)c->b_in0.p; dv = view_dirs ? (const float*)c->b_in1.p : nullptr; dr = (float*)c->b_raw.p;
    }
    RenderKernel k;
    if (pick_render_kernel(c->cfg, c->cfg.precision, false, &k)) return 1;
    if (int r = run_mlp(c, which, k, dx, dv, nullptr, dr, M, 1, 1)) return r;
    if (mem == NERF_MEM_HOST) {
        HIP_OK(hipMemcpyAsync(raw, dr, (size_t)M * 16, hipMemcpyDeviceToHost, c->stream));
        HIP_OK(hipStreamSynchronize(c->stream));
    }
    return 0;
}

int nerf_ray_marching(nerf_ctx* c, const float* raw, const float* z, int64_t N, int32_t S, const nerf_outputs* outs,
                      int mem) {
    ENTER(c);
    if (!c || !raw || !z || !outs) return fail("NULL argument");
    if (N < 0 || S <= 0) return fail("bad shape");
    if (mem == NERF_MEM_DEVICE) {
        launch_composite(raw, z, N, S, outs->rgb, outs->weights, outs->cumprod, outs->alpha, outs->rgb_samples,
                         outs->depth, c->stream);
        if (outs->z && outs->z != z)
            HIP_OK(hipMemcpyAsync(outs->z, z, (size_t)N * S * 4, hipMemcpyDeviceToDevice, c->stream));
        HIP_OK(hipGetLastError());
        return 0;
    }
    if (int r = h2d(c, c->b_raw, raw, (size_t)N * S * 16)) return r;
    if (int r = h2d(c, c->b_zc, z, (size_t)N * S * 4)) return r;
    nerf_outputs dev;
    if (int r = make_dev_outputs(c, outs, N, S, &dev)) return r;
    launch_composite((const float*)c->b_raw.p, (const float*)c->b_zc.p, N, S, dev.rgb, dev.weights, dev.cumprod,
                     dev.alpha, dev.rgb_samples, dev.depth, c->stream);
    if (dev.z) HIP_OK(hipMemcpyAsync(dev.z, c->b_zc.p, (size_t)N * S * 4, hipMemcpyDeviceToDevice, c->stream));
    HIP_OK(hipGetLastError());
    return copy_back_outputs(c, outs, &dev, N, S);
}

int nerf_render_rays(nerf_ctx* c, int which, const float* o, const float* d, const float* z, int64_t N, int32_t S,
                     const nerf_outputs* outs, int mem) {
    ENTER(c);
    if (!c || !o || !d || !z || !outs) return fail("NULL argument");
    if (which != 0 && which != 1) return fail("which must be 0 (coarse) or 1 (fine)");
    if (N < 0 || S <= 0) return fail("bad shape");
    if (mem == NERF_MEM_DEVICE) return dev_render_rays(c, which, o, d, z, N, S, *outs);
    if (int r = h2d(c, c->b_orig, o, (size_t)N * 16)) return r;
    if (int r = h2d(c, c->b_dirs, d, (size_t)N * 16)) return r;
    if (int r = h2d(c, c->b_zc, z, (size_t)N * S * 4)) return r;
    nerf_outputs dev;
    if (int r = make_dev_outputs(c, outs, N, S, &dev)) return r;
    if (int r = dev_render_rays(c, which, (const float*)c->b_orig.p, (const float*)c->b_dirs.p,
                                (const float*)c->b_zc.p, N, S, dev))
        return r;
    return copy_back_outputs(c, outs, &dev, N, S);
}

int nerf_render(nerf_ctx* c, const float* o, const float* d, int64_t N, int32_t Sc, int32_t Sf, const float* u_c,
                const float* u_f, uint64_t seed, int64_t ray_base, const nerf_outputs* outs, int mem) {
    ENTER(c);
    if (!c || !o || !d || !outs) return fail("NULL argument");
    if (N < 0 || Sc <= 0 || Sf < 0) return fail("bad shape N=%lld Sc=%d Sf=%d", (long long)N, Sc, Sf);
    const bool fine = Sf > 0 && c->net[NERF_NET_FINE].loaded;
    const int S = fine ? Sc + Sf : Sc;
    if (fine && sample_pdf_lds_bytes(Sc, Sf) > 64 * 1024) return fail("Sc=%d Sf=%d exceeds the sampler's LDS budget", Sc, Sf);
    if (mem == NERF_MEM_DEVICE) return dev_render(c, o, d, N, Sc, Sf, u_c, u_f, seed, ray_base, *outs);
    if (int r = h2d(c, c->b_orig, o, (size_t)N * 16)) return r;
    if (int r = h2d(c, c->b_dirs, d, (size_t)N * 16)) return r;
    const float *duc = nullptr, *duf = nullptr;
    if (u_c) { if (int r = h2d(c, c->b_u0, u_c, (size_t)N * Sc * 4)) return r; duc = (const float*)c->b_u0.p; }
    if (u_f && fine) { if (int r = h2d(c, c->b_u1, u_f, (size_t)N * Sf * 4)) return r; duf = (const float*)c->b_u1.p; }
    nerf_outputs dev;
    if (int r = make_dev_outputs(c, outs, N, S, &dev)) return r;
    if (int r = dev_render(c, (const float*)c->b_orig.p, (const float*)c->b_dirs.p, N, Sc, Sf, duc, duf, seed,
                           ray_base, dev))
        return r;
    return copy_back_outputs(c, outs, &dev, N, S);
}

int nerf_render_image(nerf_ctx* c, const float* c2w, float fov, int32_t H, int32_t W, int64_t ray_begin,
                      int64_t ray_count, int64_t batch, int32_t Sc, int32_t Sf, const float* u_c, const float* u_f,
                      uint64_t seed, const nerf_outputs* outs, int mem) {
    ENTER(c);
    if (!c || !c2w || !outs) return fail("NULL argument");
    if (H <= 0 || W <= 0 || Sc <= 0 || Sf < 0) return fail("bad shape");
    const long long total = (long long)H * W;
    if (ray_count <= 0) { ray_begin = 0; ray_count = total; }
    if (ray_begin < 0 || ray_begin + ray_count > total) return fail("ray slab [%lld,+%lld) outside %lld rays",
                                                                    (long long)ray_begin, (long long)ray_count, total);
    if (batch < 0) return fail("batch_size must be > 0");
    const bool fine = Sf > 0 && c->net[NERF_NET_FINE].loaded;
    const int S = fine ? Sc + Sf : Sc;
    if (fine && sample_pdf_lds_bytes(Sc, Sf) > 64 * 1024) return fail("Sc=%d Sf=%d exceeds the sampler's LDS budget", Sc, Sf);
    const long long N = ray_count;
    if (int r = sampling_ok(c)) return r;
    if (batch == 0) {
        batch = 1 << 18;
        const bool per_sample = outs->weights || outs->cumprod || outs->alpha || outs->rgb_samples || outs->z;
        if (mem == NERF_MEM_HOST && per_sample && N >= 32768) batch = ((N + 3) / 4 + 127) / 128 * 128;
    }
    if (int r = ensure(c, c->b_orig, (size_t)N * 16)) return r;
    if (int r = ensure(c, c->b_dirs, (size_t)N * 16)) return r;
    launch_raygen(c2w, fov, H, W, ray_begin, N, (float*)c->b_orig.p, (float*)c->b_dirs.p, c->stream);
    if (c->ray_space == NERF_RAYS_NDC)
        launch_rays_to_ndc((const float*)c->b_orig.p, (const float*)c->b_dirs.p, N, fov, c->ndc_near_plane, (float*)c->b_orig.p,
                           (float*)c->b_dirs.p, c->stream);
    const float *duc = u_c, *duf = u_f;
    nerf_outputs dev = *outs;
    if (mem == NERF_MEM_HOST) {
        if (u_c) { if (int r = h2d(c, c->b_u0, u_c + ray_begin * Sc, (size_t)N * Sc * 4)) return r; duc = (const float*)c->b_u0.p; }
        if (u_f && fine) { if (int r = h2d(c, c->b_u1, u_f + ray_begin * Sf, (size_t)N * Sf * 4)) return r; duf = (const float*)c->b_u1.p; }
        if (int r = make_dev_outputs(c, outs, N, S, &dev)) return r;
    } else {
        if (u_c) duc = u_c + ray_begin * Sc;
        if (u_f) duf = u_f + ray_begin * Sf;
    }
    const OutSizes sz = out_sizes(S);
    size_t k = 0;
    for (long long off = 0; off < N; off += batch, ++k) {
        const long long n = std::min<long long>(batch, N - off);
        nerf_outputs part = dev;
        for (int i = 0; i < 7; ++i) {
            float** p = out_ptrs(part, i);
            if (*p) *p += sz.per_ray[i] * off;
        }
        if (int r = dev_render(c, (const float*)c->b_orig.p + off * 4, (const float*)c->b_dirs.p + off * 4, n, Sc, Sf,
                               duc ? duc + off * Sc : nullptr, (duf && fine) ? duf + off * Sf : nullptr, seed,
                               ray_begin + off, part)) {
            if (c->copy_stream) (void)hipStreamSynchronize(c->copy_stream);
            return r;
        }
        if (mem == NERF_MEM_HOST)
            if (int r = copy_back_batch(c, outs, &dev, off, n, S, k)) { (void)hipStreamSynchronize(c->copy_stream); return r; }
    }
    if (mem == NERF_MEM_HOST && c->copy_stream) HIP_OK(hipStreamSynchronize(c->copy_stream));
    return 0;
}

int nerf_host_alloc(size_t bytes, void** out) {
    if (!out) return fail("out is NULL");
    *out = nullptr;
    if (bytes == 0) return fail("nerf_host_alloc of 0 bytes");
    HIP_OK(hipHostMalloc(out, bytes, hipHostMallocPortable));
    return 0;
}

int nerf_host_free(void* p) {
    if (!p) return 0;
    HIP_OK(hipHostFree(p));
    return 0;
}

int nerf_ctx_read_nonfinite(nerf_ctx* c, int64_t* rows) {
    if (!c || !rows) return fail("NULL argument");
    ENTER(c);
    HIP_OK(hipStreamSynchronize(c->stream));
    unsigned long long v = 0;
    HIP_OK(hipMemcpy(&v, c->nonfinite, sizeof v, hipMemcpyDeviceToHost));
    HIP_OK(hipMemset(c->nonfinite, 0, sizeof v));
    *rows = (int64_t)v;
    return 0;
}

int nerf_ctx_enable_timing(nerf_ctx* c, int on) {
    if (!c) return fail("ctx is NULL");
    HIP_OK(hipStreamSynchronize(c->stream));
    c->timing = on != 0;
    c->ev_used = 0;
    c->timed_rows = 0;
    return 0;
}

int nerf_ctx_read_timing(nerf_ctx* c, double* mlp_ms, int64_t* n_launches, int64_t* n_rows) {
    if (!c) return fail("ctx is NULL");
    HIP_OK(hipStreamSynchronize(c->stream));
    double tot = 0;
    for (size_t i = 0; i < c->ev_used; ++i) {
        float ms = 0;
        HIP_OK(hipEventElapsedTime(&ms, c->ev_pool[i].first, c->ev_pool[i].second));
        tot += ms;
    }
    if (mlp_ms) *mlp_ms = tot;
    if (n_launches) *n_launches = (int64_t)c->ev_used;
    if (n_rows) *n_rows = c->timed_rows;
    c->ev_used = 0;
    c->timed_rows = 0;
    return 0;
}

}
```

nerf_and_dietnerf_amd/csrc/nerf_kernels.h:

```cpp
#pragma once
#include <hip/hip_runtime.h>
#include <stdint.h>

namespace nerf {

constexpr int kLx = 5;
constexpr int kLd = 4;
constexpr int kHidden = 256;
constexpr int kLast = 128;
constexpr int kXyzDim = 3 + 6 * kLx;
constexpr int kDirDim = 6 * kLd;
size_t blob_floats(int lx, int ld, int n_angles);
void blob_expand_index(int lx, int ld, int n_angles, int32_t* idx, int layout_lx = kLx);

constexpr int kQuadBytes = 1024;
constexpr int kChunkQuads = 16;
constexpr int kChunkBytes = kQuadBytes * kChunkQuads;
constexpr int kRingChunks = 8;
constexpr int kRingBytes = kChunkBytes * kRingChunks;

constexpr int kQpuPE = 5;
constexpr int kQpuHid = 32;
constexpr int kQpuSkip = kQpuPE + kQpuHid;
constexpr int kQpuLast = kQpuHid + 3;
constexpr int kChunksPE = (8 * kQpuPE + 15) / 16;
constexpr int kChunksHid = (8 * kQpuHid) / 16;
constexpr int kChunksSkip = (8 * kQpuSkip + 15) / 16;
constexpr int kChunksLast = (4 * kQpuLast + 15) / 16;
constexpr int kStreamChunks = kChunksPE + 3 * kChunksHid + kChunksSkip + 3 * kChunksHid + kChunksLast;
constexpr size_t kStreamBytes = size_t(kStreamChunks) * kChunkBytes;
constexpr size_t kStreamBytesXyzF32 = size_t(142) * kChunkBytes;
constexpr size_t kStreamBytesF16 = size_t(66) * 32 * kQuadBytes;
constexpr size_t kStreamBytesF16Hi = size_t(33) * 32 * kQuadBytes;
constexpr size_t kStreamBytesF16Sig = size_t(62) * 32 * kQuadBytes;
constexpr size_t kStreamBytesF16Xyz = size_t(73) * 32 * kQuadBytes;
constexpr size_t kStreamBytesF16HiXyz = size_t(37) * 32 * kQuadBytes;

constexpr int kConstBias = 0;
constexpr int kConstBias8 = 2048;
constexpr int kConstWrgb = 2176;
constexpr int kConstBHead = 2560;
constexpr int kConstWsigH = 2564;
constexpr int kConstWsigD = 2820;
constexpr int kConstFloats = 3136;
constexpr int kConstBytes = kConstFloats * 4;

constexpr int kLdsRing = 0;
constexpr int kLdsConst = kRingBytes;
constexpr int kLdsTotal = kRingBytes + kConstBytes;

struct MlpArgs {
    const float* wstream;
    const float* wconst;
    const float* in_a;
    const float* in_b;
    const float* z;
    float* raw;
    unsigned long long* nonfinite;
    long long M;
    int S;
    int mode;
    float alpha;
    float* st_ptr[10];
    int st_ld[10];
    uint32_t* mask_ptr[10];
    int diag_wrap;
};

void launch_mlp_fp32(const MlpArgs& a, int num_cus, hipStream_t stream, bool xyz_only = false);
void mlp_fp32_set_attributes();
void pack_weights_fp32(const float* blob, int n_angles, float* stream_out , float* const_out );

void launch_mlp_f16x3(const MlpArgs& a, int num_cus, hipStream_t stream, bool single_pass = false, bool xyz_only = false);
void launch_mlp_f16x3_stash(const MlpArgs& a, int num_cus, hipStream_t stream, bool single_pass = false, bool xyz_only = false);
size_t f16_stream_bytes(int n_angles, bool hi_only);
void build_f16x3_gather(int n_angles, bool hi_only, int32_t* stream_idx ,
                        int32_t* const_idx );
void launch_repack_f16x3(const float* blob, const int32_t* stream_idx, void* stream, const int32_t* const_idx, float* cst,
                         size_t stream_bytes, hipStream_t s);
void mlp_f16x3_set_attributes();
void pack_weights_f16x3(const float* blob, int n_angles, void* stream_out, float* const_out );
void pack_weights_f16(const float* blob, int n_angles, void* stream_out, float* const_out );
void launch_mlp_f16x3_sig(const MlpArgs& a, int num_cus, hipStream_t stream);
void pack_weights_f16x3_sig(const float* blob, int n_angles, void* stream_out, float* const_out );
void build_f16x3_sig_gather(int n_angles, int32_t* stream_idx );

constexpr int kLxWide = 10;
namespace wide {
void launch_mlp_f16x3(const MlpArgs& a, int num_cus, hipStream_t stream, bool single_pass = false, bool xyz_only = false);
void launch_mlp_f16x3_stash(const MlpArgs& a, int num_cus, hipStream_t stream, bool single_pass = false, bool xyz_only = false);
void build_f16x3_gather(int n_angles, bool hi_only, int32_t* stream_idx, int32_t* const_idx);
void mlp_f16x3_set_attributes();
void pack_weights_f16x3(const float* blob, int n_angles, void* stream_out, float* const_out);
void pack_weights_f16(const float* blob, int n_angles, void* stream_out, float* const_out);
}
namespace bf16 {
void launch_mlp_bf16x3(const MlpArgs& a, int num_cus, hipStream_t stream, bool xyz_only = false);
void launch_mlp_bf16x3_sig(const MlpArgs& a, int num_cus, hipStream_t stream);
void mlp_bf16x3_set_attributes();
void pack_weights_bf16x3(const float* blob, int n_angles, void* stream_out, float* const_out );
void pack_weights_bf16x3_sig(const float* blob, int n_angles, void* stream_out, float* const_out );
void launch_repack_bf16x3(const float* blob, const int32_t* stream_idx, void* stream, size_t stream_bytes, hipStream_t s);
namespace wide {
void launch_mlp_bf16x3(const MlpArgs& a, int num_cus, hipStream_t stream, bool xyz_only = false);
void mlp_bf16x3_set_attributes();
void pack_weights_bf16x3(const float* blob, int n_angles, void* stream_out, float* const_out);
}
}
inline int pe_layout_lx(int lx) { return lx > kLx ? kLxWide : kLx; }

enum StreamKind { kF16x3, kF16Hi, kBf16x3, kF16x3Sig, kBf16x3Sig, kFp32, kStreamKinds };
enum ConstBlock { kConstFp32, kConst16, kConstBlocks };
struct StreamDesc {
    size_t bytes;
    void (*pack)(const float* blob, int n_angles, void* stream_out , float* const_out );
    ConstBlock cst;
    StreamKind table;
    bool bf16;
};
inline void render_streams(int lx, int n_angles, int which, StreamDesc d[kStreamKinds]) {
    const bool wd = lx > kLx, xyz = n_angles == 0;
    const size_t b3 = xyz ? kStreamBytesF16Xyz : kStreamBytesF16, b1 = xyz ? kStreamBytesF16HiXyz : kStreamBytesF16Hi;
    const size_t bs = !wd && !xyz && which == 0 ? kStreamBytesF16Sig : 0, bf = wd ? 0 : xyz ? kStreamBytesXyzF32 : kStreamBytes;
    d[kF16x3] = {b3, wd ? wide::pack_weights_f16x3 : pack_weights_f16x3, kConst16, kF16x3, false};
    d[kF16Hi] = {b1, wd ? wide::pack_weights_f16 : pack_weights_f16, kConst16, kF16Hi, false};
    d[kBf16x3] = {b3, wd ? bf16::wide::pack_weights_bf16x3 : bf16::pack_weights_bf16x3, kConst16, kF16x3, true};
    d[kF16x3Sig] = {bs, pack_weights_f16x3_sig, kConst16, kF16x3Sig, false};
    d[kBf16x3Sig] = {bs, bf16::pack_weights_bf16x3_sig, kConst16, kF16x3Sig, true};
    d[kFp32] = {bf, [](const float* b, int na, void* s, float* c) { pack_weights_fp32(b, na, (float*)s, c); }, kConstFp32, kFp32, false};
}
inline bool build_stream_gather(int lx, int n_angles, StreamKind k, int32_t* stream_idx, int32_t* const_idx) {
    if (k == kF16x3Sig) { build_f16x3_sig_gather(n_angles, stream_idx); return false; }
    (lx > kLx ? wide::build_f16x3_gather : build_f16x3_gather)(n_angles, k == kF16Hi, stream_idx, const_idx);
    return true;
}

void launch_mlp_f16_2t(const MlpArgs& a, int num_cus, hipStream_t stream);
void mlp_f16_2t_set_attributes();

constexpr size_t kBwdStreamBytes = size_t(73) * 32 * kQuadBytes;
constexpr int kBwdXyzLd = 64;
struct MlpBwdArgs {
    const void* wstream;
    const float* wconst;
    const float* graw;
    const uint32_t* mask_ptr[10];
    float* d_ptr[10];
    float* dx_ptr[2];
    uint16_t* rs_ptr[10];
    float* dsig;
    unsigned* gmax;
    long long Mp;
    float alpha;
    int ld, ld9;
};
void launch_mlp_bwd_f16x3(const MlpBwdArgs& a, bool dx, bool single_pass, int num_cus, hipStream_t stream,
                          bool xyz_only = false);
void mlp_bwd_f16x3_set_attributes();
void build_bwd_gather(int n_angles, bool dx, bool hi_only, int32_t* idx , int xyz_dim = kXyzDim);
void launch_repack_bwd(const float* blob, const int32_t* idx, void* stream, hipStream_t s);

void launch_raygen(const float c2w_host[16], float fov, int H, int W,
                   long long ray_begin, long long ray_count, float* orig , float* dirs,
                   hipStream_t stream);
void launch_rays_to_ndc(const float* orig, const float* dirs, long long N, float fov, float near_plane, float* out_orig,
                        float* out_dirs, hipStream_t stream);
void launch_z_values(float near_b, float far_b, bool lindisp, long long N, int S, const float* u, uint64_t seed,
                     long long ray_base, float* z, hipStream_t stream);
size_t sample_pdf_lds_bytes(int S, int Sf);
void launch_sample_pdf(const float* weights, const float* z, long long N, int S, int Sf, const float* u,
                       uint64_t seed, long long ray_base, float* z_new, float* z_merged,
                       hipStream_t stream);
void launch_composite(const float* raw, const float* z, long long N, int S, float* rgb, float* weights,
                      float* cumprod, float* alpha, float* rgb_samples, float* depth, hipStream_t stream);
void launch_composite_weights(const float* sigma, const float* z, long long N, int S, float* weights, hipStream_t stream);
void launch_posenc(const float* x, long long M, int n_enc, int passthrough, float* out, hipStream_t stream);

}
```

Before: 1.722 million.

## Compute sigma head on VALU instead of a dedicated MFMA tile

Moves the sigma output (256+dir -> 1) from a padded 32-wide MFMA tile in the last layer onto VALU dot products. These are accumulated as layer-7 activations are produced, plus the direction term, and finished with a cross-half shuffle. The last body then runs one fewer MFMA tile, and the separate sigma-only weight stream is removed, with sigma-only kernels reading the full stream. The cost is extra FMAs and LDS constant reads inside the hidden layer, along with higher register pressure.

```diff
diff --git a/nerf_and_dietnerf_amd/csrc/mlp_f16_frag.h b/nerf_and_dietnerf_amd/csrc/mlp_f16_frag.h
--- a/nerf_and_dietnerf_amd/csrc/mlp_f16_frag.h
+++ b/nerf_and_dietnerf_amd/csrc/mlp_f16_frag.h
@@ -54,9 +54,8 @@
 constexpr int kHChunksSkip = (8 * kHQpuSkip + kHCQ - 1) / kHCQ;
 constexpr int kHChunksLast = (kHTilesLast * kHQpuLast + kHCQ - 1) / kHCQ;
 constexpr int kHStreamChunks = kHChunksPE + 6 * kHChunksHid + kHChunksSkip + kHChunksLast;
-constexpr int kHChunksSig = (kHQpuLast + kHCQ - 1) / kHCQ;
-constexpr int kHStreamChunksSig = kHStreamChunks - kHChunksLast + kHChunksSig;
-static_assert(kHStreamChunksSig * (size_t)kHChunkBytes == kStreamBytesF16Sig, "sigma-only stream size mismatch");
+constexpr int kHStreamChunksSig = kHStreamChunks - kHChunksLast;
+constexpr int kHStreamChunksRgb = kHStreamChunksSig + ((kHTilesLast - 1) * kHQpuLast + kHCQ - 1) / kHCQ;
 constexpr int kFChunksPE = (8 * kHStepsPE + kHCQ - 1) / kHCQ;
 constexpr int kFChunksHid = (8 * kHStepsHid) / kHCQ;
 constexpr int kFChunksSkip = (8 * (kHStepsPE + kHStepsHid) + kHCQ - 1) / kHCQ;
@@ -69,6 +68,9 @@
 constexpr int kHConstWrgb = 2208;
 constexpr int kHConstBHead = 2592;
 constexpr int kHConstFloats = 2608;
+constexpr int kHConstWsig = 2608;
+constexpr int kHConstWsigD = 2864;
+constexpr int kHConstFloatsSv = 2896;
 
 static_assert(kHStreamChunks * (size_t)kHChunkBytes == kStreamBytesF16, "stream size mismatch");
 constexpr int kXChunksHidSig = (9 * kHQpuHid) / kHCQ;
@@ -87,8 +89,8 @@
 constexpr int kXConstWsig = 2864;
 constexpr int kXConstFloats = 3120;
 static_assert(kXConstFloats <= kConstFloats, "xyz-only constants must fit the shared LDS carve");
-enum { BODY_HIDSIG = 4, BODY_LAST0 = 5, BODY_SIG = 6 };
-static_assert(kHConstFloats <= kConstFloats, "f16x3 constants must fit the shared LDS carve");
+enum { BODY_HIDSIG = 4, BODY_LAST0 = 5 };
+static_assert(kHConstFloatsSv <= kConstFloats, "f16x3 constants must fit the shared LDS carve");
 
 template <class T>
 __device__ __forceinline__ void stream_store(T* p, const T& v) {
diff --git a/nerf_and_dietnerf_amd/csrc/mlp_f16x3.hip b/nerf_and_dietnerf_amd/csrc/mlp_f16x3.hip
--- a/nerf_and_dietnerf_amd/csrc/mlp_f16x3.hip
+++ b/nerf_and_dietnerf_amd/csrc/mlp_f16x3.hip
@@ -40,14 +40,22 @@
 __device__ unsigned long long g_stamps_h[16];
 #endif
 
-template <int BODY, bool PENDING, bool FAST, bool STASH = false, int ROT = 0>
+__device__ __forceinline__ float leaky_relu_max(float v, float alpha) {
+    const float av = alpha * v;
+    float y;
+    asm("v_max_f32 %0, %1, %2" : "=v"(y) : "v"(v), "v"(av));
+    return y;
+}
+
+template <int BODY, bool PENDING, bool FAST, bool STASH = false, int ROT = 0, bool SV = false>
 __device__ __forceinline__ void layer_body_h(Pipe& p, uint32_t lane16, uint32_t cb_h, int bias_off_bytes,
                                              float alpha, float* st_prev, float* st_cur, frag4* mk_prev_ptr,
                                              frag4* mk_cur_ptr, frag4& mk_prev, frag4& mk_cur, f32x16 (&accs)[4],
                                              frag4 (&xh)[16], frag4 (&xl)[16], frag4 (&nh)[14], frag4 (&nl)[14],
                                              const frag4 (&peh)[kHStepsPE], const frag4 (&pel)[kHStepsPE], const frag4 (&dh)[2],
                                              const frag4 (&dl)[2], float (&xc)[64], float& sigma_raw) {
-    constexpr int NU = BODY == BODY_LAST ? kHTilesLast : BODY == BODY_SIG ? 1 : BODY == BODY_HIDSIG ? 9 : BODY == BODY_LAST0 ? 4 : 8;
+    static_assert(!SV || (!FAST && !STASH && (BODY == BODY_HID || BODY == BODY_LAST)), "sigma on the VALU: the 3-pass render kernels");
+    constexpr int NU = BODY == BODY_LAST ? (SV ? kHTilesLast - 1 : kHTilesLast) : BODY == BODY_HIDSIG ? 9 : BODY == BODY_LAST0 ? 4 : 8;
     constexpr int NSTEP = BODY == BODY_PE ? kHStepsPE : (BODY == BODY_HID || BODY == BODY_HIDSIG || BODY == BODY_LAST0) ? kHStepsHid
                           : BODY == BODY_SKIP ? kHStepsPE + kHStepsHid : kHStepsHid + kHStepsDir;
     constexpr int SIG0 = BODY == BODY_HIDSIG ? 1 : 0;
@@ -81,12 +89,7 @@
         if constexpr (decltype(ic)::value < NQ) issue_read(ic);
     });
 
-    auto act = [&](float v) -> float {
-        const float av = alpha * v;
-        float y;
-        asm("v_max_f32 %0, %1, %2" : "=v"(y) : "v"(v), "v"(av));
-        return y;
-    };
+    auto act = [&](float v) -> float { return leaky_relu_max(v, alpha); };
     auto load_bias = [&](int off_bytes, f32x16& dst) {
         static_for<0, 4>([&](auto gc) {
             constexpr int g = decltype(gc)::value;
@@ -94,6 +97,14 @@
             dst[4 * g + 0] = b[0]; dst[4 * g + 1] = b[1]; dst[4 * g + 2] = b[2]; dst[4 * g + 3] = b[3];
         });
     };
+    float ws[16];
+    (void)ws;
+    auto load_wsig = [&](int t, auto gc) {
+        constexpr int g = decltype(gc)::value;
+        const f32x4 w = lds_read4(cb_h + (kHConstWsig + t * 32 + g * 8) * 4);
+        ws[4 * g + 0] = w[0]; ws[4 * g + 1] = w[1]; ws[4 * g + 2] = w[2]; ws[4 * g + 3] = w[3];
+    };
+    if constexpr (SV && BODY == BODY_LAST) static_for<0, 4>([&](auto gc) { load_wsig(7, gc); });
     float sq0 = 0.f, sq1 = 0.f;
     (void)sq0; (void)sq1;
     auto stash4 = [&](auto utc, auto rc, float y0, float y1, float* base) {
@@ -240,9 +251,11 @@
             } else if constexpr (kPend) {
                 constexpr int er = 2 * n;
                 const float y0 = act(prv[er]), y1 = act(prv[er + 1]);
+                if constexpr (SV && BODY == BODY_LAST) { sigma_raw = fmaf(ws[er], y0, sigma_raw); sigma_raw = fmaf(ws[er + 1], y1, sigma_raw); }
                 store_pair(std::integral_constant<int, 7>{}, std::integral_constant<int, er>{}, y0, y1, std::true_type{}, std::true_type{});
             } else if constexpr (kPrevS) {
                 const float y = act(prv[n]);
+                if constexpr (SV && BODY == BODY_HID) sigma_raw = fmaf(ws[n], y, sigma_raw);
                 if constexpr (kXc) {
                     xc[et * 16 + n] = y;
                     if constexpr (STASH) {
@@ -263,9 +276,10 @@
                 if constexpr (n == 8) { xh[12] = nh[12]; xl[12] = nl[12]; }
                 if constexpr (n == 9) { xh[13] = nh[13]; xl[13] = nl[13]; }
             }
+            if constexpr (SV && BODY == BODY_HID && u + 1 < NU && (n & 3) == 3) load_wsig(u, std::integral_constant<int, n / 4>{});
             if constexpr (n == (NSTEP >= 12 ? 10 : 0)) {
                 if constexpr (u + 1 < NU) load_bias(bias_off_bytes + (u + 1) * 128, nxt);
-                else if constexpr (BODY != BODY_LAST && BODY != BODY_LAST0 && BODY != BODY_SIG) load_bias(bias_off_bytes + NU * 128, nxt);
+                else if constexpr (BODY != BODY_LAST && BODY != BODY_LAST0) load_bias(bias_off_bytes + NU * 128, nxt);
             }
             if constexpr (BODY == BODY_PE && u > 0 && n == 0) {
                 static_for<0, 8>([&](auto pc) {
@@ -287,7 +301,7 @@
             }
         });
     });
-    if constexpr (BODY == BODY_LAST0) {
+    if constexpr (BODY == BODY_LAST0 || (BODY == BODY_LAST && SV)) {
         f32x16& lastacc = accs[(NU - 1 + ROT) & 3];
 #pragma unroll
         for (int r = 0; r < 16; ++r) xc[(NU - 1) * 16 + r] = act(lastacc[r]);
@@ -303,7 +317,7 @@
             if (mk_cur_ptr) stream_store(mk_cur_ptr, mk_cur);
         }
     }
-    if constexpr (BODY == BODY_LAST || BODY == BODY_SIG) {
+    if constexpr (BODY == BODY_LAST && !SV) {
         static_assert(((NU - 1 + ROT) & 3) == 0, "the sigma tile's accumulator");
         sigma_raw = accs[(NU - 1) & 3][0];
         if constexpr (STASH) { if (mk_cur_ptr) stream_store(mk_cur_ptr, mk_cur); }
@@ -332,6 +346,7 @@
 template <bool FAST, bool STASH = false, bool XYZ = false, bool SIGONLY = false>
 __device__ __forceinline__ void mlp_f16_body(const MlpArgs& a) {
     static_assert(!SIGONLY || (!FAST && !STASH && !XYZ), "the sigma-only variant is a render kernel of the 3-pass network");
+    constexpr bool kSigmaValu = !FAST && !STASH && !XYZ;
     extern __shared__ __attribute__((aligned(16))) char smem[];
     const int tid = threadIdx.x;
     const int lane = tid & 63;
@@ -345,16 +360,14 @@
     const long long ntiles = (a.M + 127) / 128;
     if ((long long)blockIdx.x >= ntiles) return;
 
-    for (int i = tid; i < (XYZ ? kXConstFloats : kHConstFloats) / 4; i += 256) {
-        const bool sig = SIGONLY && i >= kHConstBias8 / 4 && i < (kHConstBias8 + 32) / 4;
-        reinterpret_cast<f32x4*>(smem + kLdsConst)[i] =
-            reinterpret_cast<const f32x4*>(a.wconst)[sig ? i + (kHConstBiasSig - kHConstBias8) / 4 : i];
-    }
+    for (int i = tid; i < (XYZ ? kXConstFloats : kSigmaValu ? kHConstFloatsSv : kHConstFloats) / 4; i += 256)
+        reinterpret_cast<f32x4*>(smem + kLdsConst)[i] = reinterpret_cast<const f32x4*>(a.wconst)[i];
 
     Pipe p;
     p.ck = 0;
     p.src_next = 0;
-    p.n_chunks = XYZ ? (FAST ? kXFStreamChunks : kXStreamChunks) : SIGONLY ? kHStreamChunksSig : (FAST ? kFStreamChunks : kHStreamChunks);
+    p.n_chunks = XYZ ? (FAST ? kXFStreamChunks : kXStreamChunks) : SIGONLY ? kHStreamChunksSig : kSigmaValu ? kHStreamChunksRgb
+                 : (FAST ? kFStreamChunks : kHStreamChunks);
     p.wbase = reinterpret_cast<const char*>(a.wstream);
     p.voff = wave * (kHCQ / 4 * kQuadBytes) + lane * 16;
     p.wave_lds = wave * (kHCQ / 4 * kQuadBytes);
@@ -445,6 +458,16 @@
             for (int e = 0; e < 8; ++e) t8[e] = dv[n * 8 + e];
             split8<FAST>(t8, dh[n], dl[n]);
         }
+        float sig_dir = 0.f;
+        if constexpr (kSigmaValu) {
+#pragma unroll
+            for (int g = 0; g < 3; ++g) {
+                const f32x4 w = lds_read4(cb_h + (kHConstWsigD + g * 8) * 4);
+#pragma unroll
+                for (int e = 0; e < 4; ++e) sig_dir = fmaf(w[e], dv[g * 4 + e], sig_dir);
+            }
+        }
+        (void)sig_dir;
 
         auto st_of = [&](int l) -> float* {
             if constexpr (!STASH) return nullptr;
@@ -473,11 +496,12 @@
             st_cur = st_of(l);
             mk_prev_ptr = mk_cur_ptr; mk_cur_ptr = mk_of(l);
             mk_prev = mk_cur; mk_cur = frag4{0u, 0u, 0u, 0u};
+            if constexpr (kSigmaValu) { if (l == 7) sigma_raw = sig_dir; }
             if (l == 4) {
                 layer_body_h<BODY_SKIP, true, FAST, STASH>(p, lane16, cb_h, (kHConstBias + 4 * 256) * 4, a.alpha, st_prev, st_cur, mk_prev_ptr, mk_cur_ptr, mk_prev, mk_cur, accs, xh, xl, nh, nl, peh, pel, dh, dl, xc, sigma_raw);
                 STAMP(t1); acc_t[3] += t1 - t0; t0 = t1;
             } else {
-                layer_body_h<BODY_HID, true, FAST, STASH>(p, lane16, cb_h, (kHConstBias + l * 256) * 4, a.alpha, st_prev, st_cur, mk_prev_ptr, mk_cur_ptr, mk_prev, mk_cur, accs, xh, xl, nh, nl, peh, pel, dh, dl, xc, sigma_raw);
+                layer_body_h<BODY_HID, true, FAST, STASH, 0, kSigmaValu>(p, lane16, cb_h, (kHConstBias + l * 256) * 4, a.alpha, st_prev, st_cur, mk_prev_ptr, mk_cur_ptr, mk_prev, mk_cur, accs, xh, xl, nh, nl, peh, pel, dh, dl, xc, sigma_raw);
                 STAMP(t1); acc_t[2] += t1 - t0; t0 = t1;
             }
         }
@@ -491,15 +515,24 @@
             mk_prev = mk_cur; mk_cur = frag4{0u, 0u, 0u, 0u};
             layer_body_h<BODY_LAST0, true, FAST, STASH, 1>(p, lane16, cb_h, kXConstBias9 * 4, a.alpha, st_prev, st_cur, mk_prev_ptr, mk_cur_ptr, mk_prev, mk_cur, accs, xh, xl, nh, nl, peh, pel, dh, dl, xc, sigma_raw);
         } else if constexpr (SIGONLY) {
-            layer_body_h<BODY_SIG, true, FAST, STASH>(p, lane16, cb_h, kHConstBias8 * 4, a.alpha, st_prev, st_cur, mk_prev_ptr, mk_cur_ptr, mk_prev, mk_cur, accs, xh, xl, nh, nl, peh, pel, dh, dl, xc, sigma_raw);
+            static_for<0, 4>([&](auto gc) {
+                constexpr int g = decltype(gc)::value;
+                const f32x4 w = lds_read4(cb_h + (kHConstWsig + 7 * 32 + g * 8) * 4);
+#pragma unroll
+                for (int e = 0; e < 4; ++e) sigma_raw = fmaf(w[e], leaky_relu_max(accs[3][4 * g + e], a.alpha), sigma_raw);
+            });
             STAMP(t1); acc_t[4] += t1 - t0;
         } else {
             st_prev = st_cur;
             st_cur = st_of(8);
             mk_prev_ptr = mk_cur_ptr; mk_cur_ptr = mk_of(8);
             mk_prev = mk_cur; mk_cur = frag4{0u, 0u, 0u, 0u};
-            layer_body_h<BODY_LAST, true, FAST, STASH>(p, lane16, cb_h, kHConstBias8 * 4, a.alpha, st_prev, st_cur, mk_prev_ptr, mk_cur_ptr, mk_prev, mk_cur, accs, xh, xl, nh, nl, peh, pel, dh, dl, xc, sigma_raw);
+            layer_body_h<BODY_LAST, true, FAST, STASH, 0, kSigmaValu>(p, lane16, cb_h, kHConstBias8 * 4, a.alpha, st_prev, st_cur, mk_prev_ptr, mk_cur_ptr, mk_prev, mk_cur, accs, xh, xl, nh, nl, peh, pel, dh, dl, xc, sigma_raw);
             STAMP(t1); acc_t[4] += t1 - t0;
+        }
+        if constexpr (kSigmaValu) {
+            sigma_raw += __shfl_xor(sigma_raw, 32);
+            sigma_raw += lds_read4(kLdsConst + kHConstBiasSig * 4)[0];
         }
         if constexpr (SIGONLY) {
             if (valid && h == 0) {
@@ -729,7 +762,7 @@
 }
 
 template <class EmitW, class EmitC>
-static void pack_f16_map(int n_angles, bool hi_only, EmitW emit_w, EmitC emit_c, bool sig_only = false) {
+static void pack_f16_map(int n_angles, bool hi_only, EmitW emit_w, EmitC emit_c) {
     const int kd = 256 + 8 * (n_angles + 1);
     const bool xyz_only = n_angles == 0;
     const int shapes_dir[12][2] = {{kPeDim, 256}, {256, 256}, {256, 256}, {256, 256}, {kPeDim + 256, 256}, {256, 256},
@@ -746,7 +779,7 @@
     }
     size_t chunk = 0;
     auto emit_body = [&](int layer, int body) {
-        const int NU = body == BODY_LAST ? kHTilesLast : body == BODY_SIG ? 1 : body == BODY_HIDSIG ? 9 : body == BODY_LAST0 ? 4 : 8;
+        const int NU = body == BODY_LAST ? kHTilesLast : body == BODY_HIDSIG ? 9 : body == BODY_LAST0 ? 4 : 8;
         const int NSTEP = body == BODY_PE ? kHStepsPE : (body == BODY_HID || body == BODY_HIDSIG || body == BODY_LAST0) ? kHStepsHid
                           : body == BODY_SKIP ? kHStepsPE + kHStepsHid : kHStepsHid + kHStepsDir;
         const long long b0 = (long long)chunk * (kHChunkBytes / 2);
@@ -767,7 +800,7 @@
                         }
                         long long src = -1;
                         if (row >= 0) {
-                            if ((body == BODY_LAST && u == kHTilesLast - 1) || body == BODY_SIG)
+                            if (body == BODY_LAST && u == kHTilesLast - 1)
                                 src = i == 0 ? L[10].k + row : -1;
                             else if (body == BODY_HIDSIG && u == 0) src = i == 0 ? L[11].k + row : -1;
                             else if (body == BODY_HIDSIG) src = L[layer].k + (long long)row * L[layer].out + 32 * (u - 1) + i;
@@ -800,18 +833,23 @@
         for (int f = 0; f < 256; ++f) emit_c(kXConstWsig + f, L[11].k + f);
         return;
     }
-    emit_body(8, sig_only ? BODY_SIG : BODY_LAST);
+    emit_body(8, BODY_LAST);
     for (int f = 0; f < 128; ++f) emit_c(kHConstBias8 + f, L[8].b + f);
     emit_c(kHConstBiasSig + 0, L[10].b);
+    for (int f = 0; f < kHidden; ++f) emit_c(kHConstWsig + f, L[10].k + f);
+    for (int h = 0; h < 2; ++h)
+        for (int v = 0; v < 8 * kHStepsDir; ++v) {
+            const int r = h_dir_row(v, h, n_angles);
+            if (r >= 0) emit_c(kHConstWsigD + 8 * (v >> 2) + 4 * h + (v & 3), L[10].k + kHidden + r);
+        }
     for (int c = 0; c < 3; ++c)
         for (int f = 0; f < 128; ++f) emit_c(kHConstWrgb + c * 128 + f, L[9].k + f * 3 + c);
     for (int c = 0; c < 3; ++c) emit_c(kHConstBHead + c, L[9].b + c);
 }
 
-static void pack_weights_f16_impl(const float* blob, int n_angles, void* stream_out, float* const_out, bool hi_only,
-                                  bool sig_only = false) {
-    memset(stream_out, 0, sig_only ? kStreamBytesF16Sig : n_angles == 0 ? (hi_only ? kStreamBytesF16HiXyz : kStreamBytesF16Xyz)
-                                                                        : (hi_only ? kStreamBytesF16Hi : kStreamBytesF16));
+static void pack_weights_f16_impl(const float* blob, int n_angles, void* stream_out, float* const_out, bool hi_only) {
+    memset(stream_out, 0, n_angles == 0 ? (hi_only ? kStreamBytesF16HiXyz : kStreamBytesF16Xyz)
+                                        : (hi_only ? kStreamBytesF16Hi : kStreamBytesF16));
     memset(const_out, 0, kConstBytes);
     uint16_t* base = reinterpret_cast<uint16_t*>(stream_out);
     pack_f16_map(n_angles, hi_only,
@@ -821,7 +859,7 @@
                      base[ph] = hi;
                      if (pl >= 0) base[pl] = f32_to_e16(w - e16_to_f32(hi));
                  },
-                 [&](long long pos, long long src) { const_out[pos] = blob[src]; }, sig_only);
+                 [&](long long pos, long long src) { const_out[pos] = blob[src]; });
 }
 
 #if defined(NERF_BF16) && NERF_PE_LX == 5
@@ -844,9 +882,6 @@
     hipLaunchKernelGGL(repack_bf16x3_kernel, dim3((unsigned)((n + 255) / 256)), dim3(256), 0, s, blob, stream_idx,
                        reinterpret_cast<uint16_t*>(stream), n);
 }
-void pack_weights_bf16x3_sig(const float* blob, int n_angles, void* stream_out, float* const_out) {
-    pack_weights_f16_impl(blob, n_angles, stream_out, const_out, false, true);
-}
 #endif
 #ifdef NERF_BF16
 void pack_weights_bf16x3(const float* blob, int n_angles, void* stream_out, float* const_out) {
@@ -905,21 +940,6 @@
 void pack_weights_f16(const float* blob, int n_angles, void* stream_out, float* const_out) {
     pack_weights_f16_impl(blob, n_angles, stream_out, const_out, true);
 }
-#if NERF_PE_LX == 5
-void pack_weights_f16x3_sig(const float* blob, int n_angles, void* stream_out, float* const_out) {
-    pack_weights_f16_impl(blob, n_angles, stream_out, const_out, false, true);
-}
-void build_f16x3_sig_gather(int n_angles, int32_t* stream_idx) {
-    memset(stream_idx, 0, (kStreamBytesF16Sig / 2) * sizeof(int32_t));
-    pack_f16_map(n_angles, false,
-                 [&](long long ph, long long pl, long long src) {
-                     if (src < 0) return;
-                     stream_idx[ph] = (int32_t)(2 * (src + 1));
-                     stream_idx[pl] = (int32_t)(2 * (src + 1) + 1);
-                 },
-                 [](long long, long long) {}, true);
-}
-#endif
-#endif
-
-}
+#endif
+
+}
diff --git a/nerf_and_dietnerf_amd/csrc/nerf_api.hip b/nerf_and_dietnerf_amd/csrc/nerf_api.hip
--- a/nerf_and_dietnerf_amd/csrc/nerf_api.hip
+++ b/nerf_and_dietnerf_amd/csrc/nerf_api.hip
@@ -167,7 +167,7 @@
         *k = {kFp32, kConstFp32, [](const MlpArgs& a, int n, hipStream_t s, bool x) { launch_mlp_fp32(a, n, s, x); }, false};
         return 0;
     case NERF_PRECISION_F16X3:
-        if (sig) *k = {kF16x3Sig, kConst16, [](const MlpArgs& a, int n, hipStream_t s, bool) { launch_mlp_f16x3_sig(a, n, s); }, true};
+        if (sig) *k = {kF16x3, kConst16, [](const MlpArgs& a, int n, hipStream_t s, bool) { launch_mlp_f16x3_sig(a, n, s); }, true};
         else if (wide_pe) *k = {kF16x3, kConst16, [](const MlpArgs& a, int n, hipStream_t s, bool x) { wide::launch_mlp_f16x3(a, n, s, false, x); }, false};
         else *k = {kF16x3, kConst16, [](const MlpArgs& a, int n, hipStream_t s, bool x) { launch_mlp_f16x3(a, n, s, false, x); }, false};
         return 0;
@@ -179,7 +179,7 @@
         return 0;
     }
     case NERF_PRECISION_BF16X3:
-        if (sig) *k = {kBf16x3Sig, kConst16, [](const MlpArgs& a, int n, hipStream_t s, bool) { bf16::launch_mlp_bf16x3_sig(a, n, s); }, true};
+        if (sig) *k = {kBf16x3, kConst16, [](const MlpArgs& a, int n, hipStream_t s, bool) { bf16::launch_mlp_bf16x3_sig(a, n, s); }, true};
         else if (wide_pe) *k = {kBf16x3, kConst16, [](const MlpArgs& a, int n, hipStream_t s, bool x) { bf16::wide::launch_mlp_bf16x3(a, n, s, x); }, false};
         else *k = {kBf16x3, kConst16, [](const MlpArgs& a, int n, hipStream_t s, bool x) { bf16::launch_mlp_bf16x3(a, n, s, x); }, false};
         return 0;
diff --git a/nerf_and_dietnerf_amd/csrc/nerf_kernels.h b/nerf_and_dietnerf_amd/csrc/nerf_kernels.h
--- a/nerf_and_dietnerf_amd/csrc/nerf_kernels.h
+++ b/nerf_and_dietnerf_amd/csrc/nerf_kernels.h
@@ -32,7 +32,6 @@
 constexpr size_t kStreamBytesXyzF32 = size_t(142) * kChunkBytes;
 constexpr size_t kStreamBytesF16 = size_t(66) * 32 * kQuadBytes;
 constexpr size_t kStreamBytesF16Hi = size_t(33) * 32 * kQuadBytes;
-constexpr size_t kStreamBytesF16Sig = size_t(62) * 32 * kQuadBytes;
 constexpr size_t kStreamBytesF16Xyz = size_t(73) * 32 * kQuadBytes;
 constexpr size_t kStreamBytesF16HiXyz = size_t(37) * 32 * kQuadBytes;
 
@@ -82,8 +81,6 @@
 void pack_weights_f16x3(const float* blob, int n_angles, void* stream_out, float* const_out );
 void pack_weights_f16(const float* blob, int n_angles, void* stream_out, float* const_out );
 void launch_mlp_f16x3_sig(const MlpArgs& a, int num_cus, hipStream_t stream);
-void pack_weights_f16x3_sig(const float* blob, int n_angles, void* stream_out, float* const_out );
-void build_f16x3_sig_gather(int n_angles, int32_t* stream_idx );
 
 constexpr int kLxWide = 10;
 namespace wide {
@@ -99,7 +96,6 @@
 void launch_mlp_bf16x3_sig(const MlpArgs& a, int num_cus, hipStream_t stream);
 void mlp_bf16x3_set_attributes();
 void pack_weights_bf16x3(const float* blob, int n_angles, void* stream_out, float* const_out );
-void pack_weights_bf16x3_sig(const float* blob, int n_angles, void* stream_out, float* const_out );
 void launch_repack_bf16x3(const float* blob, const int32_t* stream_idx, void* stream, size_t stream_bytes, hipStream_t s);
 namespace wide {
 void launch_mlp_bf16x3(const MlpArgs& a, int num_cus, hipStream_t stream, bool xyz_only = false);
@@ -109,7 +105,7 @@
 }
 inline int pe_layout_lx(int lx) { return lx > kLx ? kLxWide : kLx; }
 
-enum StreamKind { kF16x3, kF16Hi, kBf16x3, kF16x3Sig, kBf16x3Sig, kFp32, kStreamKinds };
+enum StreamKind { kF16x3, kF16Hi, kBf16x3, kFp32, kStreamKinds };
 enum ConstBlock { kConstFp32, kConst16, kConstBlocks };
 struct StreamDesc {
     size_t bytes;
@@ -119,18 +115,16 @@
     bool bf16;
 };
 inline void render_streams(int lx, int n_angles, int which, StreamDesc d[kStreamKinds]) {
+    (void)which;
     const bool wd = lx > kLx, xyz = n_angles == 0;
     const size_t b3 = xyz ? kStreamBytesF16Xyz : kStreamBytesF16, b1 = xyz ? kStreamBytesF16HiXyz : kStreamBytesF16Hi;
-    const size_t bs = !wd && !xyz && which == 0 ? kStreamBytesF16Sig : 0, bf = wd ? 0 : xyz ? kStreamBytesXyzF32 : kStreamBytes;
+    const size_t bf = wd ? 0 : xyz ? kStreamBytesXyzF32 : kStreamBytes;
     d[kF16x3] = {b3, wd ? wide::pack_weights_f16x3 : pack_weights_f16x3, kConst16, kF16x3, false};
     d[kF16Hi] = {b1, wd ? wide::pack_weights_f16 : pack_weights_f16, kConst16, kF16Hi, false};
     d[kBf16x3] = {b3, wd ? bf16::wide::pack_weights_bf16x3 : bf16::pack_weights_bf16x3, kConst16, kF16x3, true};
-    d[kF16x3Sig] = {bs, pack_weights_f16x3_sig, kConst16, kF16x3Sig, false};
-    d[kBf16x3Sig] = {bs, bf16::pack_weights_bf16x3_sig, kConst16, kF16x3Sig, true};
     d[kFp32] = {bf, [](const float* b, int na, void* s, float* c) { pack_weights_fp32(b, na, (float*)s, c); }, kConstFp32, kFp32, false};
 }
 inline bool build_stream_gather(int lx, int n_angles, StreamKind k, int32_t* stream_idx, int32_t* const_idx) {
-    if (k == kF16x3Sig) { build_f16x3_sig_gather(n_angles, stream_idx); return false; }
     (lx > kLx ? wide::build_f16x3_gather : build_f16x3_gather)(n_angles, k == kF16Hi, stream_idx, const_idx);
     return true;
 }
```

Result: no change. 1.725 million, median of 6 (+0.2%).
